# TheStageAI/TheWhisper

Measured on NVIDIA H100. Metric: tokens_per_sec, higher is better.
Workload: dtype bf16

## Files before the change

thewhisper_b200/csrc/api.cu:

```cuda
#include <limits.h>
#include <stdarg.h>
#include <stdlib.h>
#include <string.h>

#include <chrono>
#include <map>
#include <string>
#include <tuple>
#include <vector>

#ifdef BW_F16
#define BW_RENAME_SUFFIX _f16
#define BW_API_NS bw_api_f16
#else
#define BW_RENAME_SUFFIX _bf16
#define BW_API_NS bw_api
#endif
#include "abi_rename.h"
#include "../../include/thewhisper_b200.h"
#include "decode.cuh"
#include "decode_mega_common.cuh"
#include "kernels.h"

namespace BW_NS {

static thread_local char g_err[1024] = "";
void set_error(const char* fmt, ...) {
  va_list ap;
  va_start(ap, fmt);
  vsnprintf(g_err, sizeof(g_err), fmt, ap);
  va_end(ap);
}
const char* get_error() { return g_err; }
int g_pdl = 0;
static int g_pdl_enabled = -1;

size_t word_timestamps_work_floats(int Ha, int Tcap, int S);
int word_timestamps_batch_device(cudaStream_t st, const float* align, int Ha, int Tcap, int S, const int* items_dev, const int* slot_map_dev,
                                 int map_pitch, int n, int maxT, int maxNF, double time_precision, float* work, float* out_dev);

namespace {

struct EncLayer {
  const float *ln1g, *ln1b, *bqkv, *bo, *ln2g, *ln2b, *b1, *b2;
  const bf16 *wqkv, *wo, *w1, *w2;
};
constexpr const char* kDecQuant[6] = {"wqkv", "wo", "xwq", "xwo", "w1", "w2"};
struct DecLayer {
  const float *ln1g, *ln1b, *bqkv, *bo, *ln2g, *ln2b, *xbq, *xbv, *xbo, *ln3g, *ln3b, *b1, *b2;
  const void *wqkv, *wo, *xwq, *xwo, *w1, *w2;
  const bf16 *xwk, *xwv;
  const float* sc[6] = {nullptr, nullptr, nullptr, nullptr, nullptr, nullptr};
};

struct GraphKey {
  int A, G, begin_index, ts_rules, align, variant, eos, pad, ts_begin, no_ts, key_start, scores;
  bool operator<(const GraphKey& o) const {
    return std::tie(A, G, begin_index, ts_rules, align, variant, eos, pad, ts_begin, no_ts, key_start, scores) <
           std::tie(o.A, o.G, o.begin_index, o.ts_rules, o.align, o.variant, o.eos, o.pad, o.ts_begin, o.no_ts, o.key_start, o.scores);
  }
};

}
}

using namespace BW_NS;

struct bw_engine {
  bw_config cfg;
  std::map<std::string, const void*> tensors;
  bool finalized = false;
  int D, H, S, F, V, Vp, Tmax, Spad;
  const bf16 *conv1_w = nullptr, *conv2_w = nullptr;
  const void* embed = nullptr;
  const float* embed_scale = nullptr;
  const float** wscale_tab = nullptr;
  const float *conv1_b = nullptr, *conv2_b = nullptr, *enc_pos = nullptr, *enc_lnf_g = nullptr, *enc_lnf_b = nullptr;
  const float *dec_pos = nullptr, *dec_lnf_g = nullptr, *dec_lnf_b = nullptr;
  std::vector<EncLayer> enc;
  std::vector<DecLayer> dec;
  LogmelPlan* mel_plan = nullptr;
  std::vector<int> align_pairs;
  bf16 *mel_tm = nullptr, *h1 = nullptr, *xn = nullptr, *qkv = nullptr, *vt = nullptr, *ao = nullptr, *hbuf = nullptr, *enc_out = nullptr;
  float *x_enc = nullptr, *mel_scratch = nullptr;
  unsigned* mel_max = nullptr;
  bf16 *cross_k = nullptr, *cross_v = nullptr;
  bf16 *self_k = nullptr, *self_v = nullptr;
  int *tokens = nullptr, *finished = nullptr, *pos = nullptr, *anc = nullptr, *anc_tmp = nullptr, *head_slots = nullptr;
  unsigned *done_ctr = nullptr, *xcounters = nullptr, *sup_bits = nullptr, *bsup_bits = nullptr, *sel_ctr = nullptr;
  unsigned long long* sel_best = nullptr;
  float *dx = nullptr, *dqkv = nullptr, *dattn = nullptr, *dq = nullptr, *dh = nullptr, *logits = nullptr, *part_o = nullptr,
        *part_ml = nullptr, *align = nullptr, *lse = nullptr, *ts_work = nullptr, *ts_out = nullptr;
  int *reorder_tmp = nullptr, *cand_tokens = nullptr, *ts_items = nullptr, *ts_map = nullptr;
  float *run_scores = nullptr, *cand_scores = nullptr;
  size_t align_bytes = 0;
  int A = 0, G = 1, Q = 0;
  int steps = 0;
  bw_decode_opts opts{};
  bool use_anc = false;
  int* key_start = nullptr;
  bool has_k0 = false;
  bool scores = false;
  float *sc_lp = nullptr, *sc_lmass = nullptr, *sc_nsp = nullptr;
  int* nsp_cfg = nullptr;
  bool graph_pending = false;
  std::map<GraphKey, cudaGraphExec_t> graphs;
  std::map<GraphKey, long long> graph_used;
  long long graph_tick = 0, graph_captures = 0, graph_capture_us = 0, graph_evictions = 0;
  int max_graphs = 64;
  cudaGraphExec_t cur_graph = nullptr;
  std::map<cudaGraphExec_t, int> graph_kernels;
  long long step_kernel_launches = 0;
  bool no_graph = false, simt = false, no_mega = false, no_fused_select = false;
  int mega_flags = MEGA_DEFAULT_FLAGS;
  bf16 *dbn = nullptr, *dba = nullptr, *dbh = nullptr;
  float* dpart = nullptr;
  int batch_min = 3;
  bool gemm2 = true;
  bool attn_vdirect = true;
  long long gemm2_min_rows = 1024;
  bool enc_graph = true;
  bool enc_pdl = false;
  std::map<int, cudaGraphExec_t> enc_graphs;
  std::map<int, int> enc_calls;
  int num_sms = 132;
  int pf_rows = 0;
  long long pf_part_floats = 0;
  float *pf_x = nullptr, *pf_part = nullptr;
  bf16 *pf_n = nullptr, *pf_q = nullptr, *pf_a = nullptr, *pf_h = nullptr;
  unsigned* mega_bar = nullptr;
  long long* mega_trace = nullptr;
  std::map<std::string, std::pair<void*, size_t>> buffers;
};

namespace BW_API_NS {

template <typename T>
int dalloc(bw_engine* e, const char* name, T** p, size_t count, bool zero = true) {
  const size_t bytes = count * sizeof(T);
  BW_CUDA_OK(cudaMalloc(reinterpret_cast<void**>(p), bytes ? bytes : 16));
  if (zero) BW_CUDA_OK(cudaMemset(*p, 0, bytes ? bytes : 16));
  e->buffers[name] = std::make_pair(static_cast<void*>(*p), bytes);
  return 0;
}

template <typename T>
int need(bw_engine* e, const std::string& name, const T** out) {
  auto it = e->tensors.find(name);
  BW_CHECK(it != e->tensors.end() && it->second != nullptr, "weight '%s' is not bound", name.c_str());
  *out = static_cast<const T*>(it->second);
  return 0;
}

int gemm(bw_engine* e, cudaStream_t st, const GemmA& a, const bf16* W, int B, int rows, int N, int K, const GemmEpi& epi) {
  if (e->simt) return gemm_simt(st, a, W, B, rows, N, K, epi);
  if (e->gemm2 && a.kwrap >= K && a.pitch == K && a.batch_stride == (long long)rows * K && !epi.pos && gemm_tc2_supported(B * rows, N, K) &&
      (long long)B * rows >= e->gemm2_min_rows)
    return gemm_tc2(st, a.base, W, B * rows, N, K, rows, epi, 0);
  return gemm_tc(st, a, W, B, rows, N, K, epi, 0);
}

GemmA plainA(const bf16* base, int rows, int K) {
  GemmA a;
  a.base = base;
  a.batch_stride = (long long)rows * K;
  a.pitch = K;
  a.rows_base = rows;
  a.kwrap = INT_MAX;
  return a;
}

GemmEpi plainEpi(int rows, int ld) {
  GemmEpi ep;
  ep.batch_stride = (long long)rows * ld;
  ep.row_stride = ld;
  ep.head_stride = 64;
  return ep;
}

int encode_impl(bw_engine* e, int B, cudaStream_t st) {
  const int D = e->D, S = e->S, F = e->F, H = e->H, ffn = e->cfg.ffn, nm = e->cfg.n_mels;
  {
    GemmA a;
    a.base = e->mel_tm; a.batch_stride = (long long)(F + 2) * nm; a.pitch = nm; a.rows_base = F + 2; a.kwrap = nm;
    GemmEpi ep;
    ep.bias = e->conv1_b; ep.act = 1;
    ep.out_bf16 = e->h1 + D;
    ep.batch_stride = (long long)(F + 2) * D; ep.row_stride = D;
    if (int rc = gemm(e, st, a, e->conv1_w, B, F, D, 3 * nm, ep)) return rc;
  }
  {
    GemmA a;
    a.base = e->h1; a.batch_stride = (long long)(F + 2) * D; a.pitch = 2 * D; a.rows_base = (F + 2) / 2; a.kwrap = 2 * D;
    GemmEpi ep;
    ep.bias = e->conv2_b; ep.act = 1; ep.pos = e->enc_pos;
    ep.out_f32 = e->x_enc;
    ep.batch_stride = (long long)S * D; ep.row_stride = D;
    if (int rc = gemm(e, st, a, e->conv2_w, B, S, D, 3 * D, ep)) return rc;
  }
  const float scale = 0.125f;
  (void)scale;
  for (size_t l = 0; l < e->enc.size(); ++l) {
    const EncLayer& L = e->enc[l];
    if (int rc = layernorm_bf16(st, e->x_enc, L.ln1g, L.ln1b, e->xn, B * S, D)) return rc;
    {
      GemmEpi ep = plainEpi(S, 3 * D);
      ep.bias = L.bqkv; ep.out_bf16 = e->qkv;
      if (int rc = gemm(e, st, plainA(e->xn, S, D), L.wqkv, B, S, 3 * D, D, ep)) return rc;
    }
    if (e->simt) {
      if (int rc = attn_enc_simt(st, e->qkv, e->ao, B, S, H)) return rc;
    } else {
      if (e->attn_vdirect) {
        if (int rc = attn_enc_tc(st, e->qkv, nullptr, e->ao, B, S, e->Spad, H)) return rc;
      } else {
        if (int rc = transpose_v(st, e->qkv, e->vt, B, S, e->Spad, H)) return rc;
        if (int rc = attn_enc_tc(st, e->qkv, e->vt, e->ao, B, S, e->Spad, H)) return rc;
      }
    }
    {
      GemmEpi ep = plainEpi(S, D);
      ep.bias = L.bo; ep.residual = e->x_enc; ep.out_f32 = e->x_enc;
      if (int rc = gemm(e, st, plainA(e->ao, S, D), L.wo, B, S, D, D, ep)) return rc;
    }
    if (int rc = layernorm_bf16(st, e->x_enc, L.ln2g, L.ln2b, e->xn, B * S, D)) return rc;
    {
      GemmEpi ep = plainEpi(S, ffn);
      ep.bias = L.b1; ep.act = 1; ep.out_bf16 = e->hbuf;
      if (int rc = gemm(e, st, plainA(e->xn, S, D), L.w1, B, S, ffn, D, ep)) return rc;
    }
    {
      GemmEpi ep = plainEpi(S, D);
      ep.bias = L.b2; ep.residual = e->x_enc; ep.out_f32 = e->x_enc;
      if (int rc = gemm(e, st, plainA(e->hbuf, S, ffn), L.w2, B, S, D, ffn, ep)) return rc;
    }
  }
  if (int rc = layernorm_bf16(st, e->x_enc, e->enc_lnf_g, e->enc_lnf_b, e->enc_out, B * S, D)) return rc;
  const long long per_layer = (long long)e->cfg.max_audios * H * S * 64;
  for (size_t l = 0; l < e->dec.size(); ++l) {
    const DecLayer& L = e->dec[l];
    GemmEpi ep;
    ep.batch_stride = (long long)H * S * 64; ep.row_stride = 64; ep.head_stride = (long long)S * 64;
    ep.out_bf16 = e->cross_k + l * per_layer;
    if (int rc = gemm(e, st, plainA(e->enc_out, S, D), L.xwk, B, S, D, D, ep)) return rc;
    ep.bias = L.xbv;
    ep.out_bf16 = e->cross_v + l * per_layer;
    if (int rc = gemm(e, st, plainA(e->enc_out, S, D), L.xwv, B, S, D, D, ep)) return rc;
  }
  return 0;
}

constexpr int DPART_PER_ROW = 20480;

int step_batched_impl(bw_engine* e, cudaStream_t st);
int step_batched(bw_engine* e, cudaStream_t st) {
  if (g_pdl_enabled < 0) {
    const char* ev = getenv("BW_PDL");
    g_pdl_enabled = (ev && ev[0] == '0') ? 0 : 1;
  }
  g_pdl = g_pdl_enabled;
  const int rc = step_batched_impl(e, st);
  g_pdl = 0;
  return rc;
}
int step_batched_impl(bw_engine* e, cudaStream_t st) {
  const int D = e->D, H = e->H, S = e->S, ffn = e->cfg.ffn, Tmax = e->Tmax, Q = e->Q, A = e->A, G = e->G;
  const long long self_layer = (long long)e->cfg.max_audios * e->cfg.max_beams * Tmax * D;
  const long long cross_layer = (long long)e->cfg.max_audios * H * S * 64;
  const bool w8 = e->embed_scale != nullptr;
  auto proj = [&](const bf16* in, int K, const void* W, const float* sc, int N, int* ns) {
    const DecGemmPlan pl = gemm_dec_plan(Q, N, K, e->num_sms, true, w8);
    BW_CHECK((long long)pl.ksplit * N <= DPART_PER_ROW, "batched step: %d splits x N=%d exceed the partial-sum buffer", pl.ksplit, N);
    GemmEpi ep;
    ep.out_f32 = e->dpart; ep.row_stride = N;
    *ns = pl.ksplit;
    return gemm_dec(st, in, W, sc, Q, N, K, 0, ep, pl, (long long)Q * N);
  };
  if (int rc = launch_embed(st, e->embed, e->embed_scale, e->dec_pos, e->tokens, e->pos, e->dx, Q, D, Tmax)) return rc;
  int ns = 0;
  const float* pbias = nullptr;
  for (size_t l = 0; l < e->dec.size(); ++l) {
    const DecLayer& L = e->dec[l];
    bf16* kc = e->self_k + l * self_layer;
    bf16* vc = e->self_v + l * self_layer;
    if (int rc = launch_resid_ln(st, e->dx, e->dpart, ns, (long long)Q * D, pbias, L.ln1g, L.ln1b, e->dbn, Q, D)) return rc;
    if (int rc = proj(e->dbn, D, L.wqkv, L.sc[0], 3 * D, &ns)) return rc;
    {
      SelfAttnArgs s;
      s.qkv = e->dpart; s.nsplit = ns; s.split_stride = (long long)Q * 3 * D; s.qkv_bias = L.bqkv; s.q_alpha = 0.125f;
      s.kc = kc; s.vc = vc; s.kc_w = kc; s.vc_w = vc; s.anc = e->use_anc ? e->anc : nullptr; s.out_bf16 = e->dba; s.pos = e->pos;
      s.k0 = e->has_k0 ? e->key_start : nullptr;
      s.H = H; s.D = D; s.Tmax = Tmax;
      if (int rc = launch_self_attn(st, s, Q)) return rc;
    }
    if (int rc = proj(e->dba, D, L.wo, L.sc[1], D, &ns)) return rc;
    if (int rc = launch_resid_ln(st, e->dx, e->dpart, ns, (long long)Q * D, L.bo, L.ln2g, L.ln2b, e->dbn, Q, D)) return rc;
    if (int rc = proj(e->dbn, D, L.xwq, L.sc[2], D, &ns)) return rc;
    {
      CrossAttnArgs c;
      c.q = e->dpart; c.nsplit = ns; c.split_stride = (long long)Q * D; c.q_bias = L.xbq; c.q_alpha = 0.125f;
      c.kc = e->cross_k + l * cross_layer; c.vc = e->cross_v + l * cross_layer; c.out_bf16 = e->dba;
      c.part_o = e->part_o; c.part_ml = e->part_ml; c.counters = e->xcounters;
      c.S = S; c.H = H; c.D = D; c.G = G; c.pos = e->pos;
      if (e->opts.record_alignment && e->cfg.n_align_heads > 0) {
        c.align = e->align; c.head_slots = e->head_slots + l * H; c.Ha = e->cfg.n_align_heads;
        c.Tcap = e->cfg.max_align_steps; c.step_base = e->opts.begin_index;
      }
      if (int rc = launch_cross_attn(st, c, A)) return rc;
    }
    if (int rc = proj(e->dba, D, L.xwo, L.sc[3], D, &ns)) return rc;
    if (int rc = launch_resid_ln(st, e->dx, e->dpart, ns, (long long)Q * D, L.xbo, L.ln3g, L.ln3b, e->dbn, Q, D)) return rc;
    if (int rc = proj(e->dbn, D, L.w1, L.sc[4], ffn, &ns)) return rc;
    if (int rc = launch_gelu_bias(st, e->dpart, ns, (long long)Q * ffn, L.b1, e->dbh, Q, ffn)) return rc;
    if (int rc = proj(e->dbh, ffn, L.w2, L.sc[5], D, &ns)) return rc;
    pbias = L.b2;
  }
  if (int rc = launch_resid_ln(st, e->dx, e->dpart, ns, (long long)Q * D, pbias, e->dec_lnf_g, e->dec_lnf_b, e->dbn, Q, D)) return rc;
  {
    const DecGemmPlan pl = gemm_dec_plan(Q, e->V, D, e->num_sms, false, w8);
    GemmEpi ep;
    ep.out_f32 = e->logits; ep.row_stride = e->Vp;
    if (int rc = gemm_dec(st, e->dbn, e->embed, e->embed_scale, Q, e->V, D, e->V, ep, pl, 0)) return rc;
  }
  return 0;
}

constexpr int PREFILL_ROWS = 4096;

int prefill_pass(bw_engine* e, cudaStream_t st, int t0, int n) {
  const int D = e->D, H = e->H, S = e->S, ffn = e->cfg.ffn, Tmax = e->Tmax, Q = e->Q, R = e->Q * n;
  const long long self_layer = (long long)e->cfg.max_audios * e->cfg.max_beams * Tmax * D;
  const long long cross_layer = (long long)e->cfg.max_audios * H * S * 64;
  const bool w8 = e->embed_scale != nullptr;
  auto proj = [&](const bf16* in, int K, const void* W, const float* sc, int N, int* ns) {
    const DecGemmPlan pl = gemm_dec_plan(R, N, K, e->num_sms, true, w8);
    GemmEpi ep;
    ep.out_f32 = e->pf_part; ep.row_stride = N;
    *ns = pl.ksplit;
    return gemm_dec(st, in, W, sc, R, N, K, 0, ep, pl, (long long)R * N);
  };
  if (int rc = launch_prefill_embed(st, e->embed, e->embed_scale, e->dec_pos, e->tokens, e->pf_x, Q, n, t0, D, Tmax)) return rc;
  int ns = 0;
  const float* pbias = nullptr;
  for (size_t l = 0; l < e->dec.size(); ++l) {
    const DecLayer& L = e->dec[l];
    bf16* kc = e->self_k + l * self_layer;
    bf16* vc = e->self_v + l * self_layer;
    const bool last = l + 1 == e->dec.size();
    if (int rc = launch_resid_ln(st, e->pf_x, e->pf_part, ns, (long long)R * D, pbias, L.ln1g, L.ln1b, e->pf_n, R, D)) return rc;
    if (int rc = proj(e->pf_n, D, L.wqkv, L.sc[0], 3 * D, &ns)) return rc;
    if (int rc = launch_prefill_proj_sum(st, e->pf_part, ns, (long long)R * 3 * D, L.bqkv, 3 * D, D, R, last ? nullptr : e->pf_q, kc, vc, n,
                                         t0, Tmax))
      return rc;
    if (last) break;
    if (int rc = launch_prefill_self_attn(st, e->pf_q, kc, vc, e->pf_a, Q, n, t0, H, Tmax, e->has_k0 ? e->key_start : nullptr)) return rc;
    if (int rc = proj(e->pf_a, D, L.wo, L.sc[1], D, &ns)) return rc;
    if (int rc = launch_resid_ln(st, e->pf_x, e->pf_part, ns, (long long)R * D, L.bo, L.ln2g, L.ln2b, e->pf_n, R, D)) return rc;
    if (int rc = proj(e->pf_n, D, L.xwq, L.sc[2], D, &ns)) return rc;
    if (int rc = launch_prefill_proj_sum(st, e->pf_part, ns, (long long)R * D, L.xbq, D, D, R, e->pf_q, nullptr, nullptr, n, t0, Tmax)) return rc;
    if (int rc = launch_prefill_cross_attn(st, e->pf_q, e->cross_k + l * cross_layer, e->cross_v + l * cross_layer, e->pf_a, e->A, e->G, n, S, H))
      return rc;
    if (int rc = proj(e->pf_a, D, L.xwo, L.sc[3], D, &ns)) return rc;
    if (int rc = launch_resid_ln(st, e->pf_x, e->pf_part, ns, (long long)R * D, L.xbo, L.ln3g, L.ln3b, e->pf_n, R, D)) return rc;
    if (int rc = proj(e->pf_n, D, L.w1, L.sc[4], ffn, &ns)) return rc;
    if (int rc = launch_gelu_bias(st, e->pf_part, ns, (long long)R * ffn, L.b1, e->pf_h, R, ffn)) return rc;
    if (int rc = proj(e->pf_h, ffn, L.w2, L.sc[5], D, &ns)) return rc;
    pbias = L.b2;
  }
  return 0;
}

int prefill_fits(bw_engine* e, int R) {
  const int D = e->D, ffn = e->cfg.ffn;
  const int nk[4][2] = {{3 * D, D}, {D, D}, {ffn, D}, {D, ffn}};
  for (const auto& p : nk) {
    const DecGemmPlan pl = gemm_dec_plan(R, p[0], p[1], e->num_sms, true, e->embed_scale != nullptr);
    BW_CHECK((long long)pl.ksplit * R * p[0] <= e->pf_part_floats, "bw_decode_prefill: %d splits x %d rows x N=%d exceed the partial-sum buffer",
             pl.ksplit, R, p[0]);
  }
  return 0;
}

__global__ void set_pos_kernel(int* pos, int v) { *pos = v; }

int step_impl(bw_engine* e, cudaStream_t st) {
  const int D = e->D, H = e->H, S = e->S, ffn = e->cfg.ffn, V = e->V, Tmax = e->Tmax, Q = e->Q, A = e->A, G = e->G;
  const long long self_layer0 = (long long)e->cfg.max_audios * e->cfg.max_beams * Tmax * D;
  const long long cross_layer0 = (long long)e->cfg.max_audios * H * S * 64;
  bool mega_done = false, select_done = false;
  if (!e->no_mega && !e->has_k0 && G == 1 && Q <= 8 && (int)e->dec.size() <= MEGA_MAXL) {
    MegaArgs m{};
    for (size_t l = 0; l < e->dec.size(); ++l) {
      const DecLayer& L = e->dec[l];
      MegaLayer& o = m.layers[l];
      o.ln1g = L.ln1g; o.ln1b = L.ln1b; o.bqkv = L.bqkv; o.bo = L.bo; o.ln2g = L.ln2g; o.ln2b = L.ln2b; o.xbq = L.xbq; o.xbo = L.xbo;
      o.ln3g = L.ln3g; o.ln3b = L.ln3b; o.b1 = L.b1; o.b2 = L.b2;
      o.wqkv = L.wqkv; o.wo = L.wo; o.xwq = L.xwq; o.xwo = L.xwo; o.w1 = L.w1; o.w2 = L.w2;
      o.self_k = e->self_k + l * self_layer0; o.self_v = e->self_v + l * self_layer0;
      o.cross_k = e->cross_k + l * cross_layer0; o.cross_v = e->cross_v + l * cross_layer0;
      o.head_slots = (e->opts.record_alignment && e->cfg.n_align_heads > 0) ? e->head_slots + l * H : nullptr;
    }
    m.L = (int)e->dec.size(); m.D = D; m.H = H; m.ffn = ffn; m.V = V; m.S = S; m.Tmax = Tmax; m.Q = Q;
    m.embed = e->embed; m.embed_scale = e->embed_scale; m.wscale = e->wscale_tab; m.dec_pos = e->dec_pos; m.lnf_g = e->dec_lnf_g; m.lnf_b = e->dec_lnf_b;
    m.tokens = e->tokens; m.pos = e->pos; m.ldl = e->Vp;
    m.dx = e->dx; m.dqkv = e->dqkv; m.dattn = e->dattn; m.dq = e->dq; m.dh = e->dh; m.logits = e->logits;
    m.part_o = e->part_o; m.part_ml = e->part_ml; m.bar = e->mega_bar;
    int ns = e->num_sms / (Q * H);
    const int ns_min = (S + 255) / 256;
    if (ns < ns_min) ns = ns_min;
    if (ns > XSPLIT) ns = XSPLIT;
    m.nsplit = ns;
    if (e->opts.record_alignment && e->cfg.n_align_heads > 0) {
      m.align = e->align; m.Ha = e->cfg.n_align_heads; m.Tcap = e->cfg.max_align_steps; m.step_base = e->opts.begin_index;
    }
    m.trace = e->mega_trace;
    if (!e->opts.timestamp_rules && !e->no_fused_select && !e->scores) {
      m.fuse_select = 1;
      m.suppress_bits = e->sup_bits; m.begin_suppress_bits = e->bsup_bits; m.begin_index = e->opts.begin_index;
      m.eos = e->opts.eos_token; m.pad = e->opts.pad_token; m.finished = e->finished; m.tokens_rw = e->tokens; m.pos_rw = e->pos;
      m.sel_best = e->sel_best; m.sel_ctr = e->sel_ctr;
    }
    m.flags = e->mega_flags;
    const int rc = launch_decode_mega(st, m, e->num_sms);
    if (rc == 0) {
      mega_done = true;
      select_done = m.fuse_select != 0;
    }
    else if (rc != -3) return rc;
  }
  if (!mega_done && !e->simt && Q >= e->batch_min) {
    if (int rc = step_batched(e, st)) return rc;
    mega_done = true;
  }
  if (!mega_done) {
  if (int rc = launch_embed(st, e->embed, e->embed_scale, e->dec_pos, e->tokens, e->pos, e->dx, Q, D, Tmax)) return rc;
  const long long self_layer = (long long)e->cfg.max_audios * e->cfg.max_beams * Tmax * D;
  const long long cross_layer = (long long)e->cfg.max_audios * H * S * 64;
  for (size_t l = 0; l < e->dec.size(); ++l) {
    const DecLayer& L = e->dec[l];
    bf16* kc = e->self_k + l * self_layer;
    bf16* vc = e->self_v + l * self_layer;
    for (int m0 = 0; m0 < Q; m0 += Q) {
      GemvArgs g;
      g.M = Q - m0;
      g.x = e->dx + (long long)m0 * D; g.ldx = D; g.ln_g = L.ln1g; g.ln_b = L.ln1b;
      g.W = L.wqkv; g.wscale = L.sc[0]; g.N = 3 * D; g.K = D; g.bias = L.bqkv; g.alpha = 0.125f; g.alpha_cols = D;
      g.out = e->dqkv + (long long)m0 * 3 * D; g.ldo = 3 * D;
      g.kc = kc; g.vc = vc; g.D = D; g.Tmax = Tmax; g.seq0 = m0; g.pos = e->pos;
      if (int rc = launch_gemv(st, g)) return rc;
    }
    {
      SelfAttnArgs s;
      s.qkv = e->dqkv; s.kc = kc; s.vc = vc; s.anc = e->use_anc ? e->anc : nullptr; s.out = e->dattn; s.pos = e->pos;
      s.k0 = e->has_k0 ? e->key_start : nullptr;
      s.H = H; s.D = D; s.Tmax = Tmax;
      if (int rc = launch_self_attn(st, s, Q)) return rc;
    }
    for (int m0 = 0; m0 < Q; m0 += Q) {
      GemvArgs g;
      g.M = Q - m0;
      g.x = e->dattn + (long long)m0 * D; g.ldx = D; g.W = L.wo; g.wscale = L.sc[1]; g.N = D; g.K = D; g.bias = L.bo;
      g.residual = e->dx + (long long)m0 * D; g.out = e->dx + (long long)m0 * D; g.ldo = D;
      if (int rc = launch_gemv(st, g)) return rc;
    }
    for (int m0 = 0; m0 < Q; m0 += Q) {
      GemvArgs g;
      g.M = Q - m0;
      g.x = e->dx + (long long)m0 * D; g.ldx = D; g.ln_g = L.ln2g; g.ln_b = L.ln2b;
      g.W = L.xwq; g.wscale = L.sc[2]; g.N = D; g.K = D; g.bias = L.xbq; g.alpha = 0.125f; g.alpha_cols = D;
      g.out = e->dq + (long long)m0 * D; g.ldo = D;
      if (int rc = launch_gemv(st, g)) return rc;
    }
    {
      CrossAttnArgs c;
      c.q = e->dq; c.kc = e->cross_k + l * cross_layer; c.vc = e->cross_v + l * cross_layer; c.out = e->dattn;
      c.part_o = e->part_o; c.part_ml = e->part_ml; c.counters = e->xcounters;
      c.S = S; c.H = H; c.D = D; c.G = G; c.pos = e->pos;
      if (e->opts.record_alignment && e->cfg.n_align_heads > 0) {
        c.align = e->align; c.head_slots = e->head_slots + l * H; c.Ha = e->cfg.n_align_heads;
        c.Tcap = e->cfg.max_align_steps; c.step_base = e->opts.begin_index;
      }
      if (int rc = launch_cross_attn(st, c, A)) return rc;
    }
    for (int m0 = 0; m0 < Q; m0 += Q) {
      GemvArgs g;
      g.M = Q - m0;
      g.x = e->dattn + (long long)m0 * D; g.ldx = D; g.W = L.xwo; g.wscale = L.sc[3]; g.N = D; g.K = D; g.bias = L.xbo;
      g.residual = e->dx + (long long)m0 * D; g.out = e->dx + (long long)m0 * D; g.ldo = D;
      if (int rc = launch_gemv(st, g)) return rc;
    }
    for (int m0 = 0; m0 < Q; m0 += Q) {
      GemvArgs g;
      g.M = Q - m0;
      g.x = e->dx + (long long)m0 * D; g.ldx = D; g.ln_g = L.ln3g; g.ln_b = L.ln3b;
      g.W = L.w1; g.wscale = L.sc[4]; g.N = ffn; g.K = D; g.bias = L.b1; g.act = 1;
      g.out = e->dh + (long long)m0 * ffn; g.ldo = ffn;
      if (int rc = launch_gemv(st, g)) return rc;
    }
    for (int m0 = 0; m0 < Q; m0 += Q) {
      GemvArgs g;
      g.M = Q - m0;
      g.x = e->dh + (long long)m0 * ffn; g.ldx = ffn; g.W = L.w2; g.wscale = L.sc[5]; g.N = D; g.K = ffn; g.bias = L.b2;
      g.residual = e->dx + (long long)m0 * D; g.out = e->dx + (long long)m0 * D; g.ldo = D;
      if (int rc = launch_gemv(st, g)) return rc;
    }
  }
  for (int m0 = 0; m0 < Q; m0 += Q) {
    GemvArgs g;
    g.M = Q - m0;
    g.x = e->dx + (long long)m0 * D; g.ldx = D; g.ln_g = e->dec_lnf_g; g.ln_b = e->dec_lnf_b;
    g.W = e->embed; g.wscale = e->embed_scale; g.N = V; g.K = D;
    g.out = e->logits + (long long)m0 * e->Vp; g.ldo = e->Vp;
    if (int rc = launch_gemv(st, g)) return rc;
  }
  }
  if (select_done) return 0;
  SelectArgs s;
  s.logits = e->logits; s.V = V; s.ldl = e->Vp; s.Q = Q; s.Tmax = Tmax; s.tokens = e->tokens; s.finished = e->finished; s.pos = e->pos;
  s.done_ctr = e->done_ctr; s.suppress_bits = e->sup_bits; s.begin_suppress_bits = e->bsup_bits;
  s.begin_index = e->opts.begin_index; s.eos = e->opts.eos_token; s.pad = e->opts.pad_token;
  s.ts_rules = e->opts.timestamp_rules; s.ts_begin = e->opts.timestamp_begin; s.no_ts = e->opts.no_timestamps_token;
  s.max_initial_ts = e->opts.max_initial_timestamp_index; s.out_lse = e->lse;
  if (e->scores) { s.out_lp = e->sc_lp; s.out_lmass = e->sc_lmass; s.out_nsp = e->sc_nsp; s.nsp_cfg = e->nsp_cfg; }
  if (G > 1) { s.n_cand = 2 * G; s.run_scores = e->run_scores; s.cand_scores = e->cand_scores; s.cand_tokens = e->cand_tokens; }
  return launch_select(st, s);
}

__global__ void mel_to_tm_kernel(const float* __restrict__ mel, bf16* __restrict__ out, int n_mels, int frames) {
  __shared__ float tile[32][33];
  const int b = blockIdx.z, f0 = blockIdx.x * 32, m0 = blockIdx.y * 32;
  const int tx = threadIdx.x & 31, ty = threadIdx.x >> 5;
  for (int i = ty; i < 32; i += 8) {
    const int m = m0 + i, f = f0 + tx;
    tile[i][tx] = (m < n_mels && f < frames) ? mel[((long long)b * n_mels + m) * frames + f] : 0.f;
  }
  __syncthreads();
  for (int i = ty; i < 32; i += 8) {
    const int f = f0 + i, m = m0 + tx;
    if (f < frames && m < n_mels) out[((long long)b * (frames + 2) + f + 1) * n_mels + m] = f2e(tile[tx][i]);
  }
}

__global__ void iota_anc_kernel(int* anc, int Q, int Tmax) {
  const int i = blockIdx.x * blockDim.x + threadIdx.x;
  if (i < Q * Tmax) anc[i] = i / Tmax;
}

__global__ void reorder_kernel(const int* __restrict__ anc_old, int* __restrict__ anc_new, const int* __restrict__ tok_old,
                               int* __restrict__ tok_new, const int* __restrict__ parent, const int* __restrict__ next_tok,
                               const int* __restrict__ pos_ptr, int Tmax) {
  const int i = blockIdx.x;
  const int p = parent[i];
  const int cur = *pos_ptr;
  for (int s = threadIdx.x; s < Tmax; s += blockDim.x) {
    anc_new[i * Tmax + s] = (s < cur) ? anc_old[p * Tmax + s] : i;
    int t = tok_old[p * Tmax + s];
    if (s == cur) t = next_tok[i];
    tok_new[i * Tmax + s] = t;
  }
}

}
using namespace BW_API_NS;

extern "C" {

const char* bw_last_error(void) { return BW_NS::get_error(); }
int bw_abi_version(void) { return BW_ABI_VERSION; }
int bw_runtime_flags(void) { return (g_mega_coop == 1 ? 1 : 0) | (g_pdl_enabled == 1 ? 2 : 0); }
int bw_device_count(void) {
  int n = 0;
  if (cudaGetDeviceCount(&n) != cudaSuccess) {
    cudaGetLastError();
    return 0;
  }
  return n;
}

int bw_engine_create(const bw_config* cfg, bw_engine** out) {
  BW_CHECK(cfg && out, "bw_engine_create: null argument");
  BW_CHECK(cfg->d_model == cfg->n_heads * 64, "head_dim must be 64 (d_model=%d, heads=%d)", cfg->d_model, cfg->n_heads);
  BW_CHECK(cfg->d_model % 64 == 0 && cfg->ffn % 64 == 0, "d_model and ffn must be multiples of 64");
  BW_CHECK(cfg->n_mels == 128 || cfg->n_mels == 64, "n_mels=%d unsupported (the conv stem's TMA view needs a multiple of 64)", cfg->n_mels);
  BW_CHECK(cfg->max_beams >= 1 && cfg->max_beams <= MAXG, "max_beams must be in 1..%d", MAXG);
  BW_CHECK(cfg->max_source_positions >= 1 && cfg->max_source_positions <= 1536, "max_source_positions out of range (1..1536)");
  BW_CHECK(bw_device_count() > 0, "no CUDA device: thewhisper_b200 has no CPU fallback");
  bw_engine* e = new bw_engine();
  e->cfg = *cfg;
  e->D = cfg->d_model; e->H = cfg->n_heads; e->S = cfg->max_source_positions; e->F = 2 * e->S; e->V = cfg->vocab;
  e->Tmax = cfg->max_target_positions; e->Spad = (e->S + 7) / 8 * 8;
  e->Vp = (e->V + 31) / 32 * 32;
  {
    const char* bm = getenv("BW_BATCH_MIN");
    if (bm) e->batch_min = atoi(bm);
    const char* g2 = getenv("BW_GEMM2");
    if (g2) e->gemm2 = g2[0] != '0';
    const char* eg = getenv("BW_ENC_GRAPH");
    if (eg) e->enc_graph = eg[0] != '0';
    const char* ep = getenv("BW_ENC_PDL");
    if (ep) e->enc_pdl = ep[0] != '0';
    const char* avd = getenv("BW_ATTN_VDIRECT");
    if (avd) e->attn_vdirect = avd[0] != '0';
    const char* g2r = getenv("BW_GEMM2_MIN_ROWS");
    if (g2r) e->gemm2_min_rows = atoll(g2r);
  }
  const char* ng = getenv("BW_NO_GRAPH");
  e->no_graph = ng && ng[0] == '1';
  const char* nm = getenv("BW_NO_MEGA");
  e->no_mega = nm && nm[0] == '1';
  e->no_fused_select = getenv("BW_NO_FUSED_SELECT") != nullptr;
  {
    const char* sg = getenv("BW_STEP_GRAPHS");
    if (sg) e->max_graphs = atoi(sg);
  }
  {
    const char* fl = getenv("BW_MEGA_FLAGS");
    if (fl) e->mega_flags = atoi(fl);
  }
  {
    int dev = 0, sms = 132;
    if (cudaGetDevice(&dev) == cudaSuccess && cudaDeviceGetAttribute(&sms, cudaDevAttrMultiProcessorCount, dev) == cudaSuccess) e->num_sms = sms;
  }
  const char* impl = getenv("BW_GEMM_IMPL");
  e->simt = impl && strcmp(impl, "simt") == 0;
  *out = e;
  return 0;
}

void bw_engine_destroy(bw_engine* e) {
  if (!e) return;
  for (auto& kv : e->graphs) cudaGraphExecDestroy(kv.second);
  for (auto& kv : e->enc_graphs) cudaGraphExecDestroy(kv.second);
  for (auto& kv : e->buffers) cudaFree(kv.second.first);
  logmel_plan_destroy(e->mel_plan);
  delete e;
}

int bw_engine_set_tensor(bw_engine* e, const char* name, const void* p) {
  BW_CHECK(e && name && p, "bw_engine_set_tensor: null argument");
  BW_CHECK(!e->finalized, "bw_engine_set_tensor after finalize");
  e->tensors[name] = p;
  return 0;
}

int bw_engine_set_mel_filters(bw_engine* e, const float* bank_host) {
  BW_CHECK(e && bank_host, "bw_engine_set_mel_filters: null argument");
  logmel_plan_destroy(e->mel_plan);
  e->mel_plan = nullptr;
  return logmel_plan_create_from_bank(&e->mel_plan, bank_host, e->cfg.n_mels);
}

int bw_engine_set_alignment_heads(bw_engine* e, const int32_t* pairs, int32_t n) {
  BW_CHECK(e && (pairs || n == 0), "bw_engine_set_alignment_heads: null argument");
  BW_CHECK(n == e->cfg.n_align_heads, "alignment heads: got %d pairs, config says %d", n, e->cfg.n_align_heads);
  e->align_pairs.assign(pairs, pairs + 2 * n);
  return 0;
}

int bw_engine_finalize(bw_engine* e) {
  BW_CHECK(e && !e->finalized, "bw_engine_finalize: bad engine");
  const bw_config& c = e->cfg;
  const int D = e->D, S = e->S, F = e->F, H = e->H, V = e->V, Tmax = e->Tmax, A = c.max_audios, Qm = c.max_audios * c.max_beams;
#define NEED(T, field, name) if (int rc = need<T>(e, name, &field)) return rc;
  NEED(bf16, e->conv1_w, "enc.conv1.w") NEED(float, e->conv1_b, "enc.conv1.b")
  NEED(bf16, e->conv2_w, "enc.conv2.w") NEED(float, e->conv2_b, "enc.conv2.b")
  NEED(float, e->enc_pos, "enc.pos") NEED(float, e->enc_lnf_g, "enc.lnf.g") NEED(float, e->enc_lnf_b, "enc.lnf.b")
  NEED(void, e->embed, "dec.embed") NEED(float, e->dec_pos, "dec.pos")
  NEED(float, e->dec_lnf_g, "dec.lnf.g") NEED(float, e->dec_lnf_b, "dec.lnf.b")
  e->enc.resize(c.enc_layers);
  for (int i = 0; i < c.enc_layers; ++i) {
    const std::string p = "enc." + std::to_string(i) + ".";
    EncLayer& L = e->enc[i];
    NEED(float, L.ln1g, p + "ln1.g") NEED(float, L.ln1b, p + "ln1.b") NEED(bf16, L.wqkv, p + "wqkv") NEED(float, L.bqkv, p + "bqkv")
    NEED(bf16, L.wo, p + "wo") NEED(float, L.bo, p + "bo") NEED(float, L.ln2g, p + "ln2.g") NEED(float, L.ln2b, p + "ln2.b")
    NEED(bf16, L.w1, p + "w1") NEED(float, L.b1, p + "b1") NEED(bf16, L.w2, p + "w2") NEED(float, L.b2, p + "b2")
  }
  e->dec.resize(c.dec_layers);
  for (int i = 0; i < c.dec_layers; ++i) {
    const std::string p = "dec." + std::to_string(i) + ".";
    DecLayer& L = e->dec[i];
    NEED(float, L.ln1g, p + "ln1.g") NEED(float, L.ln1b, p + "ln1.b") NEED(void, L.wqkv, p + "wqkv") NEED(float, L.bqkv, p + "bqkv")
    NEED(void, L.wo, p + "wo") NEED(float, L.bo, p + "bo") NEED(float, L.ln2g, p + "ln2.g") NEED(float, L.ln2b, p + "ln2.b")
    NEED(void, L.xwq, p + "xwq") NEED(float, L.xbq, p + "xbq") NEED(bf16, L.xwk, p + "xwk") NEED(bf16, L.xwv, p + "xwv")
    NEED(float, L.xbv, p + "xbv") NEED(void, L.xwo, p + "xwo") NEED(float, L.xbo, p + "xbo")
    NEED(float, L.ln3g, p + "ln3.g") NEED(float, L.ln3b, p + "ln3.b")
    NEED(void, L.w1, p + "w1") NEED(float, L.b1, p + "b1") NEED(void, L.w2, p + "w2") NEED(float, L.b2, p + "b2")
  }
  {
    const bool w8 = e->tensors.count("dec.embed.scale") != 0;
    std::map<std::string, bool> want;
    if (w8) NEED(float, e->embed_scale, "dec.embed.scale")
    want["dec.embed.scale"] = true;
    for (int i = 0; i < c.dec_layers; ++i) {
      for (int k = 0; k < 6; ++k) {
        const std::string n = "dec." + std::to_string(i) + "." + kDecQuant[k] + ".scale";
        want[n] = true;
        if (w8) {
          BW_CHECK(e->tensors.count(n), "int8 decoder weights: scale '%s' is not bound ('dec.embed.scale' is)", n.c_str());
          NEED(float, e->dec[i].sc[k], n)
        }
      }
    }
    for (const auto& kv : e->tensors) {
      const std::string& n = kv.first;
      if (n.size() > 6 && n.compare(n.size() - 6, 6, ".scale") == 0) {
        BW_CHECK(want.count(n), "weight '%s': only the int8 decoder matrices (dec.embed, dec.<i>.{wqkv,wo,xwq,xwo,w1,w2}) have scales", n.c_str());
        BW_CHECK(w8, "scale '%s' is bound but 'dec.embed.scale' is not: int8 decoder weights need the scales of all seven kinds", n.c_str());
      }
    }
    if (w8) {
      std::vector<const float*> tab;
      for (const DecLayer& L : e->dec) tab.insert(tab.end(), L.sc, L.sc + 6);
      if (dalloc(e, "wscale_tab", &e->wscale_tab, tab.size())) return -1;
      BW_CUDA_OK(cudaMemcpy(e->wscale_tab, tab.data(), tab.size() * sizeof(const float*), cudaMemcpyHostToDevice));
    }
  }
#undef NEED
  BW_CHECK(e->mel_plan != nullptr, "mel filter bank not set (bw_engine_set_mel_filters)");
  const size_t BS = (size_t)A * S;
  if (dalloc(e, "mel_tm", &e->mel_tm, (size_t)A * (F + 2) * c.n_mels)) return -1;
  if (dalloc(e, "mel_scratch", &e->mel_scratch, (size_t)A * F * c.n_mels)) return -1;
  if (dalloc(e, "mel_max", &e->mel_max, (size_t)A)) return -1;
  if (dalloc(e, "h1", &e->h1, (size_t)A * (F + 2) * D)) return -1;
  if (dalloc(e, "x_enc", &e->x_enc, BS * D)) return -1;
  if (dalloc(e, "xn", &e->xn, BS * D)) return -1;
  if (dalloc(e, "qkv", &e->qkv, BS * 3 * D)) return -1;
  if (dalloc(e, "vt", &e->vt, (size_t)A * H * 64 * e->Spad)) return -1;
  if (dalloc(e, "ao", &e->ao, BS * D)) return -1;
  if (dalloc(e, "hbuf", &e->hbuf, BS * c.ffn)) return -1;
  if (dalloc(e, "enc_out", &e->enc_out, BS * D)) return -1;
  if (dalloc(e, "cross_k", &e->cross_k, (size_t)c.dec_layers * A * H * S * 64, false)) return -1;
  if (dalloc(e, "cross_v", &e->cross_v, (size_t)c.dec_layers * A * H * S * 64, false)) return -1;
  if (dalloc(e, "self_k", &e->self_k, (size_t)c.dec_layers * Qm * Tmax * D, false)) return -1;
  if (dalloc(e, "self_v", &e->self_v, (size_t)c.dec_layers * Qm * Tmax * D, false)) return -1;
  if (dalloc(e, "tokens", &e->tokens, (size_t)Qm * Tmax)) return -1;
  if (dalloc(e, "tokens_tmp", &e->reorder_tmp, (size_t)Qm * Tmax + 2 * Qm)) return -1;
  if (dalloc(e, "finished", &e->finished, (size_t)Qm)) return -1;
  if (dalloc(e, "pos", &e->pos, 1)) return -1;
  if (dalloc(e, "anc", &e->anc, (size_t)Qm * Tmax)) return -1;
  if (dalloc(e, "anc_tmp", &e->anc_tmp, (size_t)Qm * Tmax)) return -1;
  if (dalloc(e, "key_start", &e->key_start, (size_t)Qm)) return -1;
  if (dalloc(e, "done_ctr", &e->done_ctr, 1)) return -1;
  if (dalloc(e, "mega_bar", &e->mega_bar, 1024)) return -1;
  {
    const char* tr = getenv("BW_MEGA_TRACE");
    if (tr && tr[0] == '1' && dalloc(e, "mega_trace", &e->mega_trace, (size_t)e->num_sms * MEGA_TRACE_N * 6)) return -1;
  }
  if (dalloc(e, "xcounters", &e->xcounters, (size_t)A * H)) return -1;
  if (dalloc(e, "sel_ctr", &e->sel_ctr, 1)) return -1;
  if (dalloc(e, "sel_best", &e->sel_best, (size_t)Qm)) return -1;
  if (dalloc(e, "sup_bits", &e->sup_bits, (size_t)(V + 31) / 32)) return -1;
  if (dalloc(e, "bsup_bits", &e->bsup_bits, (size_t)(V + 31) / 32)) return -1;
  if (dalloc(e, "dx", &e->dx, (size_t)Qm * D)) return -1;
  if (dalloc(e, "dqkv", &e->dqkv, (size_t)Qm * 3 * D)) return -1;
  if (dalloc(e, "dattn", &e->dattn, (size_t)Qm * D)) return -1;
  if (dalloc(e, "dq", &e->dq, (size_t)Qm * D)) return -1;
  if (dalloc(e, "dh", &e->dh, (size_t)Qm * c.ffn)) return -1;
  if (dalloc(e, "logits", &e->logits, (size_t)Qm * e->Vp)) return -1;
  {
    const size_t qpad = ((size_t)Qm + 127) / 128 * 128;
    if (dalloc(e, "dbn", &e->dbn, qpad * D)) return -1;
    if (dalloc(e, "dba", &e->dba, qpad * D)) return -1;
    if (dalloc(e, "dbh", &e->dbh, qpad * c.ffn)) return -1;
    if (dalloc(e, "dpart", &e->dpart, (size_t)Qm * DPART_PER_ROW)) return -1;
  }
  if (dalloc(e, "lse", &e->lse, (size_t)Qm)) return -1;
  if (dalloc(e, "sc_lp", &e->sc_lp, (size_t)Qm * e->Tmax) || dalloc(e, "sc_lmass", &e->sc_lmass, (size_t)Qm * e->Tmax) ||
      dalloc(e, "sc_nsp", &e->sc_nsp, (size_t)Qm) || dalloc(e, "nsp_cfg", &e->nsp_cfg, 2))
    return -1;
  if (dalloc(e, "run_scores", &e->run_scores, (size_t)Qm)) return -1;
  if (dalloc(e, "cand_scores", &e->cand_scores, (size_t)Qm * 16)) return -1;
  if (dalloc(e, "cand_tokens", &e->cand_tokens, (size_t)Qm * 16)) return -1;
  if (dalloc(e, "part_o", &e->part_o, (size_t)A * H * XSPLIT * c.max_beams * 64)) return -1;
  if (dalloc(e, "part_ml", &e->part_ml, (size_t)A * H * XSPLIT * c.max_beams * 2)) return -1;
  if (dalloc(e, "head_slots", &e->head_slots, (size_t)c.dec_layers * H)) return -1;
  {
    std::vector<int> hs((size_t)c.dec_layers * H, -1);
    for (int i = 0; i < c.n_align_heads && 2 * i + 1 < (int)e->align_pairs.size(); ++i) {
      const int l = e->align_pairs[2 * i], h = e->align_pairs[2 * i + 1];
      BW_CHECK(l >= 0 && l < c.dec_layers && h >= 0 && h < H, "alignment head (%d,%d) out of range", l, h);
      hs[(size_t)l * H + h] = i;
    }
    BW_CUDA_OK(cudaMemcpy(e->head_slots, hs.data(), hs.size() * sizeof(int), cudaMemcpyHostToDevice));
  }
  if (c.n_align_heads > 0) {
    BW_CHECK((int)e->align_pairs.size() == 2 * c.n_align_heads, "alignment heads not set");
    if (dalloc(e, "align", &e->align, (size_t)Qm * c.n_align_heads * c.max_align_steps * S)) return -1;
    if (dalloc(e, "ts_map", &e->ts_map, (size_t)A * c.max_align_steps)) return -1;
    if (dalloc(e, "ts_work", &e->ts_work, (size_t)A * word_timestamps_work_floats(c.n_align_heads, c.max_align_steps, S), false)) return -1;
    if (dalloc(e, "ts_out", &e->ts_out, (size_t)A * (c.max_align_steps + 8))) return -1;
    if (dalloc(e, "ts_items", &e->ts_items, (size_t)A * 3)) return -1;
  }
  e->finalized = true;
  return 0;
}

int bw_engine_buffer(bw_engine* e, const char* name, void** p, size_t* bytes) {
  BW_CHECK(e && name && p, "bw_engine_buffer: null argument");
  auto it = e->buffers.find(name);
  BW_CHECK(it != e->buffers.end(), "bw_engine_buffer: unknown buffer '%s'", name);
  *p = it->second.first;
  if (bytes) *bytes = it->second.second;
  return 0;
}

int bw_logmel(bw_engine* e, const float* pcm, int32_t B, int32_t n_samples, float* mel_f32_out, void* stream) {
  BW_CHECK(e && e->finalized && pcm, "bw_logmel: bad arguments");
  BW_CHECK(B >= 1 && B <= e->cfg.max_audios, "bw_logmel: B=%d outside 1..%d", B, e->cfg.max_audios);
  BW_CHECK(n_samples == e->F * 160, "bw_logmel: n_samples=%d, expected %d for this chunk length", n_samples, e->F * 160);
  return logmel(static_cast<cudaStream_t>(stream), e->mel_plan, pcm, B, n_samples, e->F, e->mel_tm, mel_f32_out, e->mel_scratch, e->mel_max);
}

int bw_logmel_long(bw_engine* e, const float* pcm, int32_t B, int32_t n_samples, float* mel_f32_out, void* stream) {
  BW_CHECK(e && e->finalized && pcm && mel_f32_out, "bw_logmel_long: bad arguments");
  BW_CHECK(B >= 1 && B <= e->cfg.max_audios, "bw_logmel_long: B=%d outside 1..%d", B, e->cfg.max_audios);
  BW_CHECK(n_samples >= 400, "bw_logmel_long: n_samples=%d below one 400-sample frame", n_samples);
  return logmel_long(static_cast<cudaStream_t>(stream), e->mel_plan, pcm, B, n_samples, mel_f32_out, e->mel_max);
}

int bw_set_mel(bw_engine* e, const float* mel, int32_t B, void* stream) {
  BW_CHECK(e && e->finalized && mel, "bw_set_mel: bad arguments");
  BW_CHECK(B >= 1 && B <= e->cfg.max_audios, "bw_set_mel: B=%d outside 1..%d", B, e->cfg.max_audios);
  dim3 grid((e->F + 31) / 32, (e->cfg.n_mels + 31) / 32, B);
  mel_to_tm_kernel<<<grid, 256, 0, static_cast<cudaStream_t>(stream)>>>(mel, e->mel_tm, e->cfg.n_mels, e->F);
  BW_CUDA_OK(cudaGetLastError());
  return 0;
}

static int encode_pdl(bw_engine* e, int B, cudaStream_t st) {
  if (!e->enc_pdl) return encode_impl(e, B, st);
  if (g_pdl_enabled < 0) {
    const char* ev = getenv("BW_PDL");
    g_pdl_enabled = (ev && ev[0] == '0') ? 0 : 1;
  }
  g_pdl = g_pdl_enabled;
  const int rc = encode_impl(e, B, st);
  g_pdl = 0;
  return rc;
}

int bw_encode(bw_engine* e, int32_t B, void* stream) {
  BW_CHECK(e && e->finalized, "bw_encode: engine not finalized");
  BW_CHECK(B >= 1 && B <= e->cfg.max_audios, "bw_encode: B=%d outside 1..%d", B, e->cfg.max_audios);
  cudaStream_t st = static_cast<cudaStream_t>(stream);
  if (e->no_graph || !e->enc_graph || e->simt) return encode_pdl(e, B, st);
  auto it = e->enc_graphs.find(B);
  if (it == e->enc_graphs.end()) {
    if (e->enc_calls[B]++ == 0) return encode_pdl(e, B, st);
    cudaStream_t cs;
    BW_CUDA_OK(cudaStreamCreateWithFlags(&cs, cudaStreamNonBlocking));
    cudaGraph_t graph = nullptr;
    cudaGraphExec_t exec = nullptr;
    for (int attempt = 0; attempt < 2 && !exec; ++attempt) {
      BW_CUDA_OK(cudaStreamBeginCapture(cs, cudaStreamCaptureModeThreadLocal));
      const int rc = encode_pdl(e, B, cs);
      cudaError_t ce = cudaStreamEndCapture(cs, &graph);
      if (rc == 0 && ce == cudaSuccess) ce = cudaGraphInstantiate(&exec, graph, 0);
      if (graph) cudaGraphDestroy(graph);
      graph = nullptr;
      if (rc == 0 && ce == cudaSuccess) break;
      exec = nullptr;
      cudaGetLastError();
      if (attempt == 0 && g_pdl_enabled == 1) {
        g_pdl_enabled = 0;
        continue;
      }
      break;
    }
    cudaStreamDestroy(cs);
    if (!exec) {
      e->enc_graph = false;
      return encode_pdl(e, B, st);
    }
    it = e->enc_graphs.emplace(B, exec).first;
  }
  BW_CUDA_OK(cudaGraphLaunch(it->second, st));
  return 0;
}

int bw_decode_begin(bw_engine* e, int32_t A, int32_t G, const int32_t* prompt, int32_t plen, const bw_decode_opts* opts, void* stream) {
  return bw_decode_begin_key_start(e, A, G, prompt, plen, opts, nullptr, stream);
}

int bw_decode_begin_key_start(bw_engine* e, int32_t A, int32_t G, const int32_t* prompt, int32_t plen, const bw_decode_opts* opts,
                              const int32_t* key_start, void* stream) {
  BW_CHECK(e && e->finalized && prompt && opts, "bw_decode_begin: bad arguments");
  BW_CHECK(A >= 1 && A <= e->cfg.max_audios && G >= 1 && G <= e->cfg.max_beams, "bw_decode_begin: A=%d G=%d out of range", A, G);
  BW_CHECK(plen >= 1 && plen <= e->Tmax, "bw_decode_begin: prompt_len=%d out of range", plen);
  BW_CHECK(opts->begin_index >= 1 && opts->begin_index <= plen, "bw_decode_begin: begin_index=%d outside 1..prompt_len", opts->begin_index);
  bool has_k0 = false;
  if (key_start)
    for (int a = 0; a < A; ++a) {
      BW_CHECK(key_start[a] >= 0 && key_start[a] < opts->begin_index, "bw_decode_begin: key_start[%d]=%d outside 0..begin_index-1 = 0..%d", a,
               key_start[a], opts->begin_index - 1);
      has_k0 |= key_start[a] > 0;
    }
  cudaStream_t st = static_cast<cudaStream_t>(stream);
  e->A = A; e->G = G; e->Q = A * G; e->opts = *opts; e->use_anc = G > 1; e->steps = 0; e->has_k0 = has_k0;
  const int Q = e->Q, Tmax = e->Tmax, V = e->V;
  std::vector<int> k0v((size_t)Q, 0);
  if (has_k0) {
    for (int q = 0; q < Q; ++q) k0v[q] = key_start[q / G];
    BW_CUDA_OK(cudaMemcpyAsync(e->key_start, k0v.data(), sizeof(int) * Q, cudaMemcpyHostToDevice, st));
  }
  std::vector<int> tok((size_t)Q * Tmax, opts->pad_token);
  for (int q = 0; q < Q; ++q) memcpy(&tok[(size_t)q * Tmax], prompt + (size_t)q * plen, sizeof(int) * plen);
  BW_CUDA_OK(cudaMemcpyAsync(e->tokens, tok.data(), tok.size() * sizeof(int), cudaMemcpyHostToDevice, st));
  std::vector<unsigned> bits((V + 31) / 32, 0u), bbits((V + 31) / 32, 0u);
  for (int i = 0; i < opts->n_suppress; ++i) {
    const int t = opts->suppress_tokens[i];
    if (t >= 0 && t < V) bits[t >> 5] |= 1u << (t & 31);
  }
  for (int i = 0; i < opts->n_begin_suppress; ++i) {
    const int t = opts->begin_suppress_tokens[i];
    if (t >= 0 && t < V) bbits[t >> 5] |= 1u << (t & 31);
  }
  BW_CUDA_OK(cudaMemcpyAsync(e->sup_bits, bits.data(), bits.size() * sizeof(unsigned), cudaMemcpyHostToDevice, st));
  BW_CUDA_OK(cudaMemcpyAsync(e->bsup_bits, bbits.data(), bbits.size() * sizeof(unsigned), cudaMemcpyHostToDevice, st));
  BW_CUDA_OK(cudaMemsetAsync(e->finished, 0, sizeof(int) * Q, st));
  BW_CUDA_OK(cudaMemsetAsync(e->pos, 0, sizeof(int), st));
  BW_CUDA_OK(cudaMemsetAsync(e->done_ctr, 0, sizeof(unsigned), st));
  BW_CUDA_OK(cudaMemsetAsync(e->xcounters, 0, sizeof(unsigned) * e->cfg.max_audios * e->H, st));
  iota_anc_kernel<<<(Q * Tmax + 255) / 256, 256, 0, st>>>(e->anc, Q, Tmax);
  BW_CUDA_OK(cudaGetLastError());
  BW_CUDA_OK(cudaStreamSynchronize(st));
  e->cur_graph = nullptr;
  e->scores = false;
  e->graph_pending = !e->no_graph;
  return 0;
}

static int acquire_step_graph(bw_engine* e) {
  e->graph_pending = false;
  const bw_decode_opts* opts = &e->opts;
  const int A = e->A, G = e->G;
  {
    GraphKey key{A, G, opts->begin_index, opts->timestamp_rules * 4 + (opts->max_initial_timestamp_index + 1) * 8, opts->record_alignment,
                 e->mega_flags * 4 + (e->no_mega ? 1 : 0) + (e->no_fused_select ? 2 : 0),
                 opts->eos_token, opts->pad_token, opts->timestamp_begin, opts->no_timestamps_token, e->has_k0 ? 1 : 0, e->scores ? 1 : 0};
    auto it = e->graphs.find(key);
    if (it == e->graphs.end()) {
      while (e->max_graphs > 0 && (int)e->graphs.size() >= e->max_graphs) {
        auto lru = e->graph_used.begin();
        for (auto u = e->graph_used.begin(); u != e->graph_used.end(); ++u)
          if (u->second < lru->second) lru = u;
        auto g = e->graphs.find(lru->first);
        e->graph_kernels.erase(g->second);
        cudaGraphExecDestroy(g->second);
        e->graphs.erase(g);
        e->graph_used.erase(lru);
        ++e->graph_evictions;
      }
      const auto t_capture = std::chrono::steady_clock::now();
      cudaStream_t cs;
      BW_CUDA_OK(cudaStreamCreateWithFlags(&cs, cudaStreamNonBlocking));
      cudaGraph_t graph = nullptr;
      for (int attempt = 0; attempt < 2; ++attempt) {
        BW_CUDA_OK(cudaStreamBeginCapture(cs, cudaStreamCaptureModeThreadLocal));
        const int rc = step_impl(e, cs);
        const cudaError_t ce = cudaStreamEndCapture(cs, &graph);
        if (rc == 0 && ce == cudaSuccess) break;
        if (graph) cudaGraphDestroy(graph);
        graph = nullptr;
        cudaGetLastError();
        if (attempt == 0 && (g_mega_coop == 1 || g_pdl_enabled == 1)) {
          g_mega_coop = 0;
          g_pdl_enabled = 0;
          continue;
        }
        cudaStreamDestroy(cs);
        if (rc == 0) set_error("cudaStreamEndCapture: %s", cudaGetErrorString(ce));
        return -1;
      }
      int n_kernel_nodes = 0;
      {
        size_t nn = 0;
        if (cudaGraphGetNodes(graph, nullptr, &nn) == cudaSuccess && nn > 0) {
          std::vector<cudaGraphNode_t> nodes(nn);
          if (cudaGraphGetNodes(graph, nodes.data(), &nn) == cudaSuccess) {
            for (size_t i = 0; i < nn; ++i) {
              cudaGraphNodeType ty;
              if (cudaGraphNodeGetType(nodes[i], &ty) == cudaSuccess && ty == cudaGraphNodeTypeKernel) ++n_kernel_nodes;
            }
          }
        }
      }
      cudaGraphExec_t exec = nullptr;
      BW_CUDA_OK(cudaGraphInstantiate(&exec, graph, 0));
      cudaGraphDestroy(graph);
      e->graph_kernels[exec] = n_kernel_nodes;
      cudaStreamDestroy(cs);
      it = e->graphs.emplace(key, exec).first;
      ++e->graph_captures;
      e->graph_capture_us +=
          std::chrono::duration_cast<std::chrono::microseconds>(std::chrono::steady_clock::now() - t_capture).count();
    }
    e->graph_used[key] = ++e->graph_tick;
    e->cur_graph = it->second;
  }
  return 0;
}

int bw_decode_run(bw_engine* e, int32_t n_steps, void* stream) {
  BW_CHECK(e && e->finalized && e->Q > 0, "bw_decode_run: no decode in progress");
  BW_CHECK(n_steps >= 0 && n_steps <= e->Tmax - e->steps, "bw_decode_run: %d steps from position %d would run past the last position %d",
           n_steps, e->steps, e->Tmax - 1);
  cudaStream_t st = static_cast<cudaStream_t>(stream);
  if (n_steps > 0 && e->graph_pending)
    if (int rc = acquire_step_graph(e)) return rc;
  for (int i = 0; i < n_steps; ++i, ++e->steps) {
    if (e->cur_graph) {
      BW_CUDA_OK(cudaGraphLaunch(e->cur_graph, st));
      e->step_kernel_launches += e->graph_kernels[e->cur_graph];
    } else {
      if (int rc = step_impl(e, st)) return rc;
    }
  }
  return 0;
}

int bw_decode_prefill(bw_engine* e, int32_t n_positions, int32_t max_rows_per_pass, void* stream) {
  BW_CHECK(e && e->finalized && e->Q > 0, "bw_decode_prefill: no decode in progress");
  BW_CHECK(e->steps == 0, "bw_decode_prefill: %d decoder steps have run since bw_decode_begin; the prefill must come first", e->steps);
  BW_CHECK(n_positions >= 1 && n_positions <= e->opts.begin_index - 1, "bw_decode_prefill: n_positions=%d outside 1..begin_index-1 = 1..%d",
           n_positions, e->opts.begin_index - 1);
  BW_CHECK(max_rows_per_pass == 0 || max_rows_per_pass >= e->Q, "bw_decode_prefill: max_rows_per_pass=%d is below the %d sequences of one position",
           max_rows_per_pass, e->Q);
  const bw_config& c = e->cfg;
  if (!e->pf_h) {
    const long long qm = (long long)c.max_audios * c.max_beams;
    e->pf_rows = (int)(qm * e->Tmax < PREFILL_ROWS ? qm * e->Tmax : (qm > PREFILL_ROWS ? qm : PREFILL_ROWS));
    const size_t rows = (size_t)e->pf_rows;
    const int widest = c.ffn > 3 * e->D ? c.ffn : 3 * e->D;
    e->pf_part_floats = (long long)rows * widest > (long long)e->num_sms * 128 * 256 ? (long long)rows * widest : (long long)e->num_sms * 128 * 256;
    const char* names[5] = {"pf_x", "pf_part", "pf_n", "pf_q", "pf_a"};
    for (const char* nm : names) {
      auto it = e->buffers.find(nm);
      if (it != e->buffers.end()) {
        cudaFree(it->second.first);
        e->buffers.erase(it);
      }
    }
    if (dalloc(e, "pf_x", &e->pf_x, rows * e->D, false) || dalloc(e, "pf_part", &e->pf_part, (size_t)e->pf_part_floats, false) ||
        dalloc(e, "pf_n", &e->pf_n, rows * e->D, false) || dalloc(e, "pf_q", &e->pf_q, rows * e->D, false) ||
        dalloc(e, "pf_a", &e->pf_a, rows * e->D, false) || dalloc(e, "pf_h", &e->pf_h, rows * c.ffn, false))
      return -1;
  }
  cudaStream_t st = static_cast<cudaStream_t>(stream);
  const int rows = (max_rows_per_pass > 0 && max_rows_per_pass < e->pf_rows) ? max_rows_per_pass : e->pf_rows;
  const int per = rows / e->Q;
  for (int t0 = 0; t0 < n_positions; t0 += per)
    if (int rc = prefill_fits(e, e->Q * (n_positions - t0 < per ? n_positions - t0 : per))) return rc;
  for (int t0 = 0; t0 < n_positions; t0 += per) {
    const int n = n_positions - t0 < per ? n_positions - t0 : per;
    if (int rc = prefill_pass(e, st, t0, n)) return rc;
  }
  set_pos_kernel<<<1, 1, 0, st>>>(e->pos, n_positions);
  BW_CUDA_OK(cudaGetLastError());
  e->steps = n_positions;
  return 0;
}

int bw_decode_scores_enable(bw_engine* e, int32_t nospeech_pos, int32_t nospeech_token, void* stream) {
  BW_CHECK(e && e->finalized && e->Q > 0, "bw_decode_scores_enable: no decode in progress");
  BW_CHECK(e->steps == 0, "bw_decode_scores_enable: a step or prefill has run since bw_decode_begin; scores must be enabled before it");
  BW_CHECK(nospeech_pos >= -1 && nospeech_pos <= e->opts.begin_index - 1, "bw_decode_scores_enable: nospeech_pos=%d outside -1..begin_index-1 = -1..%d",
           nospeech_pos, e->opts.begin_index - 1);
  BW_CHECK(nospeech_token >= 0 && nospeech_token < e->V, "bw_decode_scores_enable: nospeech_token=%d outside 0..%d", nospeech_token, e->V - 1);
  cudaStream_t st = static_cast<cudaStream_t>(stream);
  const int cfg[2] = {nospeech_pos, nospeech_token};
  BW_CUDA_OK(cudaMemcpyAsync(e->nsp_cfg, cfg, sizeof(cfg), cudaMemcpyHostToDevice, st));
  BW_CUDA_OK(cudaMemsetAsync(e->sc_lp, 0, sizeof(float) * e->Q * e->Tmax, st));
  BW_CUDA_OK(cudaMemsetAsync(e->sc_lmass, 0, sizeof(float) * e->Q * e->Tmax, st));
  BW_CUDA_OK(cudaMemsetAsync(e->sc_nsp, 0, sizeof(float) * e->Q, st));
  BW_CUDA_OK(cudaStreamSynchronize(st));
  e->scores = true;
  return 0;
}

int bw_decode_read_scores(bw_engine* e, float* lp_host, float* lmass_host, float* nsp_host, void* stream) {
  BW_CHECK(e && e->finalized && e->Q > 0 && e->scores, "bw_decode_read_scores: no decode with scores in progress");
  cudaStream_t st = static_cast<cudaStream_t>(stream);
  const size_t n = (size_t)e->Q * e->Tmax;
  if (lp_host) BW_CUDA_OK(cudaMemcpyAsync(lp_host, e->sc_lp, sizeof(float) * n, cudaMemcpyDeviceToHost, st));
  if (lmass_host) BW_CUDA_OK(cudaMemcpyAsync(lmass_host, e->sc_lmass, sizeof(float) * n, cudaMemcpyDeviceToHost, st));
  if (nsp_host) BW_CUDA_OK(cudaMemcpyAsync(nsp_host, e->sc_nsp, sizeof(float) * e->Q, cudaMemcpyDeviceToHost, st));
  BW_CUDA_OK(cudaStreamSynchronize(st));
  return 0;
}

long long bw_decode_kernel_launches(bw_engine* e) { return e ? e->step_kernel_launches : -1; }

int bw_decode_graph_stats(bw_engine* e, int64_t* out) {
  BW_CHECK(e && out, "bw_decode_graph_stats: bad arguments");
  out[0] = e->graph_captures;
  out[1] = e->graph_capture_us;
  out[2] = (int64_t)e->graphs.size();
  out[3] = e->graph_evictions;
  return 0;
}

int bw_decode_read(bw_engine* e, int32_t* tokens_host, int32_t* finished_host, int32_t* pos_host, void* stream) {
  BW_CHECK(e && e->finalized && e->Q > 0, "bw_decode_read: no decode in progress");
  cudaStream_t st = static_cast<cudaStream_t>(stream);
  if (tokens_host) BW_CUDA_OK(cudaMemcpyAsync(tokens_host, e->tokens, sizeof(int) * e->Q * e->Tmax, cudaMemcpyDeviceToHost, st));
  if (finished_host) BW_CUDA_OK(cudaMemcpyAsync(finished_host, e->finished, sizeof(int) * e->Q, cudaMemcpyDeviceToHost, st));
  if (pos_host) BW_CUDA_OK(cudaMemcpyAsync(pos_host, e->pos, sizeof(int), cudaMemcpyDeviceToHost, st));
  BW_CUDA_OK(cudaStreamSynchronize(st));
  return 0;
}

int bw_decode_reorder(bw_engine* e, const int32_t* parent_host, const int32_t* next_token_host, void* stream) {
  BW_CHECK(e && e->finalized && e->Q > 0 && parent_host && next_token_host, "bw_decode_reorder: bad arguments");
  cudaStream_t st = static_cast<cudaStream_t>(stream);
  const int Q = e->Q, Tmax = e->Tmax;
  int* d_parent = e->reorder_tmp + (size_t)e->cfg.max_audios * e->cfg.max_beams * Tmax;
  int* d_next = d_parent + Q;
  BW_CUDA_OK(cudaMemcpyAsync(d_parent, parent_host, sizeof(int) * Q, cudaMemcpyHostToDevice, st));
  BW_CUDA_OK(cudaMemcpyAsync(d_next, next_token_host, sizeof(int) * Q, cudaMemcpyHostToDevice, st));
  reorder_kernel<<<Q, 128, 0, st>>>(e->anc, e->anc_tmp, e->tokens, e->reorder_tmp, d_parent, d_next, e->pos, Tmax);
  BW_CUDA_OK(cudaGetLastError());
  BW_CUDA_OK(cudaMemcpyAsync(e->anc, e->anc_tmp, sizeof(int) * Q * Tmax, cudaMemcpyDeviceToDevice, st));
  BW_CUDA_OK(cudaMemcpyAsync(e->tokens, e->reorder_tmp, sizeof(int) * Q * Tmax, cudaMemcpyDeviceToDevice, st));
  BW_CUDA_OK(cudaStreamSynchronize(st));
  return 0;
}

int bw_decode_beam_step(bw_engine* e, const float* run_scores_host, float* cand_scores_host, int32_t* cand_tokens_host, void* stream) {
  BW_CHECK(e && e->finalized && e->Q > 0 && e->G > 1, "bw_decode_beam_step: no beam decode in progress");
  BW_CHECK(run_scores_host && cand_scores_host && cand_tokens_host, "bw_decode_beam_step: null pointer");
  cudaStream_t st = static_cast<cudaStream_t>(stream);
  const int Q = e->Q, nc = 2 * e->G;
  BW_CUDA_OK(cudaMemcpyAsync(e->run_scores, run_scores_host, sizeof(float) * Q, cudaMemcpyHostToDevice, st));
  if (int rc = bw_decode_run(e, 1, stream)) return rc;
  BW_CUDA_OK(cudaMemcpyAsync(cand_scores_host, e->cand_scores, sizeof(float) * Q * nc, cudaMemcpyDeviceToHost, st));
  BW_CUDA_OK(cudaMemcpyAsync(cand_tokens_host, e->cand_tokens, sizeof(int) * Q * nc, cudaMemcpyDeviceToHost, st));
  BW_CUDA_OK(cudaStreamSynchronize(st));
  return 0;
}

static int word_timestamps_impl(bw_engine* e, int32_t n, const int32_t* audio, const int32_t* slot_map, int32_t map_pitch, const int32_t* n_tokens,
                                const int32_t* num_frames, double time_precision, float* out_host, int32_t out_pitch, void* stream) {
  BW_CHECK(e && e->finalized && (audio || slot_map) && n_tokens && num_frames && out_host, "bw_word_timestamps: bad arguments");
  BW_CHECK(e->cfg.n_align_heads > 0 && e->align, "bw_word_timestamps: engine built without alignment heads");
  BW_CHECK(n >= 1 && n <= e->cfg.max_audios, "bw_word_timestamps: n=%d outside 1..%d", n, e->cfg.max_audios);
  const int Tcap = e->cfg.max_align_steps, Qm = e->cfg.max_audios * e->cfg.max_beams;
  std::vector<int> items((size_t)n * 3), map;
  int maxT = 0, maxNF = 0;
  for (int i = 0; i < n; ++i) {
    BW_CHECK(n_tokens[i] >= 1 && n_tokens[i] <= Tcap, "bw_word_timestamps: n_tokens=%d outside 1..%d", n_tokens[i], Tcap);
    BW_CHECK(num_frames[i] >= 1 && num_frames[i] <= e->S, "bw_word_timestamps: num_frames=%d outside 1..%d", num_frames[i], e->S);
    BW_CHECK(out_pitch >= n_tokens[i] + 1, "bw_word_timestamps: out_pitch=%d too small for %d tokens", out_pitch, n_tokens[i]);
    if (audio) BW_CHECK(audio[i] >= 0 && audio[i] < Qm, "bw_word_timestamps: slot index out of range");
    items[3 * i] = audio ? audio[i] : 0; items[3 * i + 1] = n_tokens[i]; items[3 * i + 2] = num_frames[i];
    maxT = n_tokens[i] > maxT ? n_tokens[i] : maxT;
    maxNF = num_frames[i] > maxNF ? num_frames[i] : maxNF;
  }
  cudaStream_t st = static_cast<cudaStream_t>(stream);
  if (slot_map) {
    BW_CHECK(map_pitch >= maxT, "bw_word_timestamps_gather: map_pitch=%d smaller than %d tokens", map_pitch, maxT);
    map.assign((size_t)n * Tcap, 0);
    for (int i = 0; i < n; ++i)
      for (int t = 0; t < n_tokens[i]; ++t) {
        const int sl = slot_map[(size_t)i * map_pitch + t];
        BW_CHECK(sl >= 0 && sl < Qm, "bw_word_timestamps_gather: slot %d out of range", sl);
        map[(size_t)i * Tcap + t] = sl;
      }
    BW_CUDA_OK(cudaMemcpyAsync(e->ts_map, map.data(), map.size() * sizeof(int), cudaMemcpyHostToDevice, st));
  }
  BW_CUDA_OK(cudaMemcpyAsync(e->ts_items, items.data(), items.size() * sizeof(int), cudaMemcpyHostToDevice, st));
  if (int rc = word_timestamps_batch_device(st, e->align, e->cfg.n_align_heads, Tcap, e->S, e->ts_items, slot_map ? e->ts_map : nullptr, Tcap, n, maxT,
                                            maxNF, time_precision, e->ts_work, e->ts_out))
    return rc;
  BW_CUDA_OK(cudaMemcpy2DAsync(out_host, (size_t)out_pitch * sizeof(float), e->ts_out, (size_t)(Tcap + 8) * sizeof(float),
                               (size_t)(maxT + 1) * sizeof(float), n, cudaMemcpyDeviceToHost, st));
  BW_CUDA_OK(cudaStreamSynchronize(st));
  return 0;
}

int bw_word_timestamps_batch(bw_engine* e, int32_t n, const int32_t* audio, const int32_t* n_tokens, const int32_t* num_frames,
                             double time_precision, float* out_host, int32_t out_pitch, void* stream) {
  BW_CHECK(audio, "bw_word_timestamps_batch: null argument");
  return word_timestamps_impl(e, n, audio, nullptr, 0, n_tokens, num_frames, time_precision, out_host, out_pitch, stream);
}

int bw_word_timestamps_gather(bw_engine* e, int32_t n, const int32_t* slot_map, int32_t map_pitch, const int32_t* n_tokens,
                              const int32_t* num_frames, double time_precision, float* out_host, int32_t out_pitch, void* stream) {
  BW_CHECK(slot_map, "bw_word_timestamps_gather: null argument");
  return word_timestamps_impl(e, n, nullptr, slot_map, map_pitch, n_tokens, num_frames, time_precision, out_host, out_pitch, stream);
}

int bw_word_timestamps(bw_engine* e, int32_t audio, int32_t n_tokens, int32_t num_frames, double time_precision, float* out_host,
                       void* stream) {
  return bw_word_timestamps_batch(e, 1, &audio, &n_tokens, &num_frames, time_precision, out_host, n_tokens + 1, stream);
}

int bw_op_gemm(const void* A, const void* W, int32_t M, int32_t N, int32_t K, const float* bias, float alpha, int32_t act,
               const float* residual, void* out, int32_t out_is_f32, int32_t impl, int32_t force_bn, void* stream) {
  BW_CHECK(A && W && out, "bw_op_gemm: null pointer");
  GemmEpi ep = plainEpi(M, N);
  ep.bias = bias; ep.alpha = alpha; ep.act = act; ep.residual = residual;
  if (out_is_f32) ep.out_f32 = static_cast<float*>(out);
  else ep.out_bf16 = static_cast<bf16*>(out);
  const GemmA a = plainA(static_cast<const bf16*>(A), M, K);
  cudaStream_t st = static_cast<cudaStream_t>(stream);
  if (impl == 1) return gemm_simt(st, a, static_cast<const bf16*>(W), 1, M, N, K, ep);
  if (impl == 2) return gemm_tc2(st, static_cast<const bf16*>(A), static_cast<const bf16*>(W), M, N, K, M, ep, force_bn);
  return gemm_tc(st, a, static_cast<const bf16*>(W), 1, M, N, K, ep, force_bn);
}

int bw_op_gemm_splitk(const void* A, const void* W, int32_t M, int32_t N, int32_t K, int32_t n_valid, int32_t ksplit, int32_t force_bn,
                      float* out_partials, int32_t* ksplit_used, void* stream) {
  BW_CHECK(A && W && out_partials && ksplit_used, "bw_op_gemm_splitk: null pointer");
  GemmEpi ep = plainEpi(M, N);
  ep.out_f32 = out_partials;
  ep.n_valid = (n_valid > 0 && n_valid < N) ? n_valid : 0;
  *ksplit_used = gemm_tc_ksplit(K, ksplit);
  return gemm_tc_split(static_cast<cudaStream_t>(stream), plainA(static_cast<const bf16*>(A), M, K), static_cast<const bf16*>(W), 1, M, N, K, ep,
                       force_bn, ksplit, (long long)M * N);
}

int bw_op_gemm_dec(const void* X, const void* W, int32_t Q, int32_t N, int32_t K, int32_t n_valid, int32_t want_split, float* out_partials,
                   int32_t* ksplit_used, void* stream) {
  BW_CHECK(X && W && out_partials && ksplit_used, "bw_op_gemm_dec: null pointer");
  int dev = 0, sms = 132;
  if (cudaGetDevice(&dev) == cudaSuccess) cudaDeviceGetAttribute(&sms, cudaDevAttrMultiProcessorCount, dev);
  const DecGemmPlan pl = gemm_dec_plan(Q, N, K, sms, want_split != 0);
  *ksplit_used = pl.ksplit;
  GemmEpi ep;
  ep.out_f32 = out_partials; ep.row_stride = N;
  return gemm_dec(static_cast<cudaStream_t>(stream), static_cast<const bf16*>(X), W, nullptr, Q, N, K, n_valid, ep, pl, (long long)Q * N);
}

int bw_op_gelu_bias(const float* partials, int32_t nsplit, const float* bias, void* h_bf16, int32_t Q, int32_t N, void* stream) {
  BW_CHECK(partials && bias && h_bf16 && nsplit >= 1, "bw_op_gelu_bias: bad arguments");
  return launch_gelu_bias(static_cast<cudaStream_t>(stream), partials, nsplit, (long long)Q * N, bias, static_cast<bf16*>(h_bf16), Q, N);
}

int bw_op_resid_ln(float* x, const float* partials, int32_t nsplit, const float* bias, const float* ln_g, const float* ln_b, void* y_bf16,
                   int32_t Q, int32_t D, void* stream) {
  BW_CHECK(x && (nsplit == 0 || partials) && (!y_bf16 || (ln_g && ln_b)), "bw_op_resid_ln: null pointer");
  return launch_resid_ln(static_cast<cudaStream_t>(stream), x, partials, nsplit, (long long)Q * D, bias, ln_g, ln_b, static_cast<bf16*>(y_bf16), Q, D);
}

int bw_op_attn_enc(const void* qkv, void* vt_scratch, void* out, int32_t B, int32_t S, int32_t H, int32_t impl, void* stream) {
  BW_CHECK(qkv && out, "bw_op_attn_enc: null pointer");
  cudaStream_t st = static_cast<cudaStream_t>(stream);
  if (impl == 1) return attn_enc_simt(st, static_cast<const bf16*>(qkv), static_cast<bf16*>(out), B, S, H);
  BW_CHECK(vt_scratch, "bw_op_attn_enc: vt_scratch required for the tensor-core path");
  const int Spad = (S + 7) / 8 * 8;
  if (impl == 3) return attn_enc_tc(st, static_cast<const bf16*>(qkv), nullptr, static_cast<bf16*>(out), B, S, Spad, H);
  if (int rc = transpose_v(st, static_cast<const bf16*>(qkv), static_cast<bf16*>(vt_scratch), B, S, Spad, H)) return rc;
  return attn_enc_tc(st, static_cast<const bf16*>(qkv), static_cast<const bf16*>(vt_scratch), static_cast<bf16*>(out), B, S, Spad, H);
}

int bw_op_layernorm(const float* x, const float* g, const float* b, void* out, int32_t out_is_f32, int32_t rows, int32_t D, void* stream) {
  BW_CHECK(x && g && b && out, "bw_op_layernorm: null pointer");
  cudaStream_t st = static_cast<cudaStream_t>(stream);
  return out_is_f32 ? layernorm_f32(st, x, g, b, static_cast<float*>(out), rows, D)
                    : layernorm_bf16(st, x, g, b, static_cast<bf16*>(out), rows, D);
}

int bw_op_gemv(const float* x, const float* ln_g, const float* ln_b, const void* W, int32_t M, int32_t N, int32_t K, const float* bias,
               float alpha, int32_t act, const float* residual, float* out, void* stream) {
  BW_CHECK(x && W && out, "bw_op_gemv: null pointer");
  GemvArgs g;
  g.x = x; g.ldx = K; g.ln_g = ln_g; g.ln_b = ln_b; g.W = static_cast<const bf16*>(W); g.N = N; g.K = K; g.M = M;
  g.bias = bias; g.alpha = alpha; g.alpha_cols = (alpha != 1.0f) ? N : 0; g.act = act; g.residual = residual; g.out = out; g.ldo = N;
  return launch_gemv(static_cast<cudaStream_t>(stream), g);
}

static int mega_plan(int32_t Q, int32_t D, int32_t ffn, int32_t num_sms, int32_t smem_optin, int32_t static_smem, int64_t* out, int esz) {
  BW_CHECK(out && Q >= 1 && D > 0 && ffn > 0 && num_sms > 0 && smem_optin > static_smem, "bw_op_mega_plan: bad arguments");
  int p0_off = 0;
  const size_t smem = mega::mega_smem_plan(Q <= 1 ? 1 : 2, D, ffn, num_sms, true, (size_t)(smem_optin - static_smem), &p0_off, esz);
  out[0] = (int64_t)smem;
  out[1] = p0_off;
  return smem ? 0 : -3;
}

int bw_op_mega_plan(int32_t Q, int32_t D, int32_t ffn, int32_t num_sms, int32_t smem_optin, int32_t static_smem, int64_t* out) {
  return mega_plan(Q, D, ffn, num_sms, smem_optin, static_smem, out, 2);
}

int bw_op_mega_plan_w8(int32_t Q, int32_t D, int32_t ffn, int32_t num_sms, int32_t smem_optin, int32_t static_smem, int64_t* out) {
  return mega_plan(Q, D, ffn, num_sms, smem_optin, static_smem, out, 1);
}

}
```

thewhisper_b200/csrc/decode.cuh:

```cuda
#pragma once
#include "common.cuh"

namespace BW_NS {

struct GemvArgs {
  const float* x = nullptr;
  int ldx = 0;
  const float* ln_g = nullptr;
  const float* ln_b = nullptr;
  const void* W = nullptr;
  const float* wscale = nullptr;
  int N = 0, K = 0, M = 0;
  const float* bias = nullptr;
  float alpha = 1.0f;
  int alpha_cols = 0;
  int act = 0;
  const float* residual = nullptr;
  float* out = nullptr;
  int ldo = 0;
  bf16* kc = nullptr;
  bf16* vc = nullptr;
  int D = 0, Tmax = 0, seq0 = 0;
  const int* pos = nullptr;
};

struct SelfAttnArgs {
  const float* qkv = nullptr;
  const bf16* kc = nullptr;
  const bf16* vc = nullptr;
  const int* anc = nullptr;
  float* out = nullptr;
  bf16* out_bf16 = nullptr;
  const int* pos = nullptr;
  const int* k0 = nullptr;
  int H = 0, D = 0, Tmax = 0;
  bf16* kc_w = nullptr;
  bf16* vc_w = nullptr;
  int nsplit = 0;
  long long split_stride = 0;
  const float* qkv_bias = nullptr;
  float q_alpha = 1.0f;
};

constexpr int XSPLIT = 12;
constexpr int MAXG = 8;

struct CrossAttnArgs {
  const float* q = nullptr;
  const bf16* kc = nullptr;
  const bf16* vc = nullptr;
  float* out = nullptr;
  bf16* out_bf16 = nullptr;
  float* part_o = nullptr;
  float* part_ml = nullptr;
  unsigned* counters = nullptr;
  int S = 0, H = 0, D = 0, G = 1;
  float* align = nullptr;
  int align_slot = -1;
  const int* head_slots = nullptr;
  int Ha = 0, Tcap = 0, step_base = 0;
  const int* pos = nullptr;
  int nsplit = 0;
  long long split_stride = 0;
  const float* q_bias = nullptr;
  float q_alpha = 1.0f;
};

struct SelectArgs {
  const float* logits = nullptr;
  int V = 0, Q = 0, Tmax = 0, ldl = 0;
  int* tokens = nullptr;
  int* finished = nullptr;
  int* pos = nullptr;
  unsigned* done_ctr = nullptr;
  const unsigned* suppress_bits = nullptr;
  const unsigned* begin_suppress_bits = nullptr;
  int begin_index = 0;
  int eos = 0, pad = 0;
  int ts_rules = 0, ts_begin = 0, no_ts = 0, max_initial_ts = -1;
  float* out_lse = nullptr;
  float* out_lp = nullptr;
  float* out_lmass = nullptr;
  float* out_nsp = nullptr;
  const int* nsp_cfg = nullptr;
  int n_cand = 0;
  const float* run_scores = nullptr;
  float* cand_scores = nullptr;
  int* cand_tokens = nullptr;
};

struct MegaLayer {
  const float *ln1g, *ln1b, *bqkv, *bo, *ln2g, *ln2b, *xbq, *xbo, *ln3g, *ln3b, *b1, *b2;
  const void *wqkv, *wo, *xwq, *xwo, *w1, *w2;
  bf16 *self_k, *self_v;
  const bf16 *cross_k, *cross_v;
  const int* head_slots;
};

constexpr int MEGA_MAXL = 32;
constexpr int MEGA_DEFAULT_FLAGS = 64;
constexpr int MEGA_TRACE_N = 264;

struct MegaArgs {
  MegaLayer layers[MEGA_MAXL];
  int L, D, H, ffn, V, S, Tmax, Q;
  int ldl;
  const void* embed;
  const float* dec_pos;
  const float *lnf_g, *lnf_b;
  const int* tokens;
  const int* pos;
  float *dx, *dqkv, *dattn, *dq, *dh, *logits;
  float *part_o, *part_ml;
  unsigned* bar;
  int nsplit;
  float* align;
  int Ha, Tcap, step_base;
  long long* trace;
  int flags;
  int fuse_select;
  const unsigned* suppress_bits;
  const unsigned* begin_suppress_bits;
  int begin_index, eos, pad;
  int* finished;
  int* tokens_rw;
  int* pos_rw;
  unsigned long long* sel_best;
  unsigned* sel_ctr;
  int p0_off;
  const float* const* wscale;
  const float* embed_scale;
};

int launch_decode_mega(cudaStream_t st, const MegaArgs& a, int num_sms);
extern int g_mega_coop;
int launch_gemv(cudaStream_t st, const GemvArgs& a);
int launch_embed(cudaStream_t st, const void* E, const float* Es, const float* P, const int* tokens, const int* pos, float* x, int Q, int D, int Tmax);
int launch_self_attn(cudaStream_t st, const SelfAttnArgs& a, int Q);
int launch_cross_attn(cudaStream_t st, const CrossAttnArgs& a, int A);
int launch_select(cudaStream_t st, const SelectArgs& a);
int launch_resid_ln(cudaStream_t st, float* x, const float* part, int nsplit, long long split_stride, const float* bias, const float* g,
                    const float* b, bf16* y, int Q, int D);


int launch_prefill_embed(cudaStream_t st, const void* E, const float* Es, const float* P, const int* tokens, float* x, int Q, int n, int t0,
                         int D, int Tmax);
int launch_prefill_proj_sum(cudaStream_t st, const float* part, int nsplit, long long split_stride, const float* bias, int N, int D, int R,
                            bf16* qout, bf16* kc, bf16* vc, int n, int t0, int Tmax);
int launch_prefill_self_attn(cudaStream_t st, const bf16* q, const bf16* kc, const bf16* vc, bf16* out, int Q, int n, int t0, int H, int Tmax,
                             const int* k0 = nullptr);
int launch_prefill_cross_attn(cudaStream_t st, const bf16* q, const bf16* kc, const bf16* vc, bf16* out, int A, int G, int n, int S, int H);

}
```

thewhisper_b200/csrc/decode_mega.cu:

```cuda
#include "decode_mega_common.cuh"

namespace BW_NS {

namespace {

using namespace mega;


constexpr unsigned V_NOTRACE = 1;

__device__ __noinline__ void wait_timeout(const char* what, unsigned a0, unsigned a1) {
  printf("[bw] decode_mega: %s timed out (block %d thread %d: %u %u)\n", what, blockIdx.x, threadIdx.x, a0, a1);
  __trap();
}
template <unsigned VAR>
struct GridBar {
  static constexpr bool TRACE = !(VAR & V_NOTRACE);
  unsigned* ctr;
  unsigned nblocks;
  unsigned epoch;
  long long* trace;
  __device__ __forceinline__ void arrive() {
    if (threadIdx.x == MT - 1) {
      if (TRACE && trace && epoch < MEGA_TRACE_N) trace[((long long)blockIdx.x * MEGA_TRACE_N + epoch) * 2] = global_ns();
      red_release_add(ctr, 1u);
    }
  }
  __device__ __forceinline__ void wait() {
    if (threadIdx.x == MT - 1) {
      const unsigned target = (epoch + 1) * nblocks;
      if (ld_acquire_u32(ctr) < target) {
        const long long t0 = clock64();
        while (ld_acquire_u32(ctr) < target) {
          if (clock64() - t0 > (1ll << 32)) {
            printf("[bw] decode_mega: grid barrier %u timed out (block %d)\n", epoch, blockIdx.x);
            __trap();
          }
        }
      }
      if (TRACE && trace && epoch < MEGA_TRACE_N) trace[((long long)blockIdx.x * MEGA_TRACE_N + epoch) * 2 + 1] = global_ns();
    }
    ++epoch;
    __syncthreads();
  }
  __device__ __forceinline__ void sync() {
    __syncthreads();
    arrive();
    wait();
  }
};

struct GemvDesc {
  const uint8_t* W;
  const float* scale;
  const float* bias;
  int N, K, R;
  int n0, nend;
  bool lm;
  const float* src;
  const float *lng, *lnb;
  float* out;
  int ldo;
  const float* residual;
  int act;
  float alpha;
  int alpha_cols;
  bf16 *kc, *vc;
};

__device__ __forceinline__ void split_rows(GemvDesc& d) {
  const int rc = (d.N + (int)gridDim.x - 1) / (int)gridDim.x;
  d.R = (rc + MW - 1) / MW;
  d.n0 = min(d.N, (int)blockIdx.x * rc);
  d.nend = min(d.N, d.n0 + rc);
}
template <unsigned VAR, bool W8>
__device__ __forceinline__ GemvDesc make_desc(const MegaArgs& a, const MegaLayer* layers, int l, int g, int pos) {
  GemvDesc d;
  d.scale = nullptr;
  if constexpr (W8) d.scale = l >= a.L ? a.embed_scale : a.wscale[l * 6 + g];
  d.lng = d.lnb = nullptr;
  d.residual = nullptr;
  d.act = 0;
  d.alpha = 1.f;
  d.alpha_cols = 0;
  d.kc = d.vc = nullptr;
  d.N = d.K = d.ldo = a.D;
  d.lm = false;
  if (l >= a.L) {
    d.W = static_cast<const uint8_t*>(a.embed); d.bias = nullptr; d.N = a.V; d.R = 2; d.n0 = 0; d.nend = a.V; d.lm = true; d.src = a.dx; d.lng = a.lnf_g; d.lnb = a.lnf_b; d.out = a.logits; d.ldo = a.ldl;
    return d;
  }
  const MegaLayer& L = layers[l];
  switch (g) {
    case 0:
      d.W = static_cast<const uint8_t*>(L.wqkv); d.bias = L.bqkv; d.N = 3 * a.D; d.src = a.dx; d.lng = L.ln1g; d.lnb = L.ln1b; d.out = a.dqkv; d.ldo = 3 * a.D;
      d.alpha = 0.125f; d.alpha_cols = a.D; d.kc = L.self_k; d.vc = L.self_v;
      break;
    case 1:
      d.W = static_cast<const uint8_t*>(L.wo); d.bias = L.bo; d.src = a.dattn; d.out = a.dx; d.residual = a.dx;
      break;
    case 2:
      d.W = static_cast<const uint8_t*>(L.xwq); d.bias = L.xbq; d.src = a.dx; d.lng = L.ln2g; d.lnb = L.ln2b; d.out = a.dq; d.alpha = 0.125f; d.alpha_cols = a.D;
      break;
    case 3:
      d.W = static_cast<const uint8_t*>(L.xwo); d.bias = L.xbo; d.src = a.part_o; d.out = a.dx; d.residual = a.dx;
      break;
    case 4:
      d.W = static_cast<const uint8_t*>(L.w1); d.bias = L.b1; d.N = a.ffn; d.src = a.dx; d.lng = L.ln3g; d.lnb = L.ln3b; d.out = a.dh; d.ldo = a.ffn; d.act = 1;
      break;
    default:
      d.W = static_cast<const uint8_t*>(L.w2); d.bias = L.b2; d.K = a.ffn; d.src = a.dh; d.out = a.dx; d.residual = a.dx;
      break;
  }
  split_rows(d);
  return d;
}

struct Pre {
  float bias;
  float scale;
  float4 g, b;
};

template <int ESZ>
__device__ __forceinline__ void issue_slabs(const GemvDesc& d, uint8_t* region, uint64_t* cbar) {
  if (threadIdx.x == DMA_T && d.n0 < d.nend) {
    const uint32_t bytes = (uint32_t)(d.nend - d.n0) * d.K * ESZ;
    mbar_arrive_expect_tx(cbar, bytes);
    if constexpr (ESZ == 2) bulk_g2s(region, reinterpret_cast<const bf16*>(d.W) + (long long)d.n0 * d.K, bytes, cbar);
    else bulk_g2s(region, d.W + (long long)d.n0 * d.K, bytes, cbar);
  }
}

template <bool W8>
__device__ __forceinline__ void prefetch_phase(const GemvDesc& d, Pre& p, uint8_t* pool, uint64_t* wbar, int gw, int warp, int lane) {
  constexpr int ESZ = W8 ? 1 : 2;
  int n;
  if (d.lm) {
    n = gw * d.R;
    if (n < d.N) issue_rows<ESZ>(pool + (size_t)warp * d.R * d.K * ESZ, wbar, d.W, d.K, d.R, n, d.N, lane);
  } else {
    n = d.n0 + warp * d.R;
  }
  const int r_sel = lane >> 3;
  p.bias = (d.bias && (lane & 7) < 2 && r_sel < d.R && n + r_sel < d.nend) ? d.bias[n + r_sel] : 0.f;
  if constexpr (W8) p.scale = (!d.lm && (lane & 7) < 2 && r_sel < d.R && n + r_sel < d.nend) ? d.scale[n + r_sel] : 1.f;
  const int k = threadIdx.x * 4;
  if (d.lng && k < d.K) {
    p.g = *reinterpret_cast<const float4*>(d.lng + k);
    p.b = *reinterpret_cast<const float4*>(d.lnb + k);
  }
}

template <int MB>
__device__ __forceinline__ void merge_xattn(float* xs, const GemvDesc& d, const MegaArgs& a, int M) {
  constexpr int XC = 6;
  static_assert(MAXD <= (MT - 32) * 4 && XSPLIT <= 16, "one float4 per staging thread and sequence; one lane per split");
  const int K = d.K, nsplit = a.nsplit;
  const int k = threadIdx.x * 4, sp_l = threadIdx.x & 15;
  const bool have = k < K;
#pragma unroll 1
  for (int m = 0; m < MB; ++m) {
    const int hb = (m * a.H + (k >> 6)) * nsplit;
    const float* po_base = a.part_o + hb * 64 + (k & 63);
    const bool live = have && m < M;
    float pm = -INFINITY, pl = 0.f;
    float4 po[XC];
    if (live && sp_l < nsplit) {
      const float2 v = __ldcg(reinterpret_cast<const float2*>(a.part_ml) + hb + sp_l);
      pm = v.x;
      pl = v.y;
    }
#pragma unroll
    for (int sp = 0; sp < XC; ++sp) {
      po[sp] = make_float4(0.f, 0.f, 0.f, 0.f);
      if (live && sp < nsplit) po[sp] = __ldcg(reinterpret_cast<const float4*>(po_base + sp * 64));
    }
    if (m == 0) asm volatile("bar.arrive 2, %0;" ::"n"(MT) : "memory");
    float mx = pl > 0.f ? pm : -INFINITY;
#pragma unroll
    for (int s = 8; s >= 1; s >>= 1) mx = fmaxf(mx, __shfl_xor_sync(0xffffffffu, mx, s));
    float lsum = 0.f;
    float4 o = make_float4(0.f, 0.f, 0.f, 0.f);
    for (int sp0 = 0;;) {
#pragma unroll
      for (int sp = 0; sp < XC; ++sp) {
        const float sm = __shfl_sync(0xffffffffu, pm, sp0 + sp, 16), sl = __shfl_sync(0xffffffffu, pl, sp0 + sp, 16);
        if (sp0 + sp < nsplit && sl > 0.f) {
          const float w = __expf(sm - mx);
          lsum = fmaf(sl, w, lsum);
          o.x = fmaf(po[sp].x, w, o.x);
          o.y = fmaf(po[sp].y, w, o.y);
          o.z = fmaf(po[sp].z, w, o.z);
          o.w = fmaf(po[sp].w, w, o.w);
        }
      }
      sp0 += XC;
      if (sp0 >= nsplit) break;
#pragma unroll
      for (int sp = 0; sp < XC; ++sp)
        if (live && sp0 + sp < nsplit) po[sp] = __ldcg(reinterpret_cast<const float4*>(po_base + (sp0 + sp) * 64));
    }
    if (!have) continue;
    float4 v = make_float4(0.f, 0.f, 0.f, 0.f);
    if (m < M) {
      v = make_float4(o.x / lsum, o.y / lsum, o.z / lsum, o.w / lsum);
      float* row = a.dattn + m * K;
      if (k >= d.n0 && k < d.nend) row[k] = v.x;
      if (k + 1 >= d.n0 && k + 1 < d.nend) row[k + 1] = v.y;
      if (k + 2 >= d.n0 && k + 2 < d.nend) row[k + 2] = v.z;
      if (k + 3 >= d.n0 && k + 3 < d.nend) row[k + 3] = v.w;
    }
    *reinterpret_cast<float4*>(xs + m * K + k) = v;
  }
}

__device__ __forceinline__ void stage_sync() { asm volatile("bar.sync 1, %0;" ::"n"(MT - 32) : "memory"); }
__device__ __forceinline__ void stage_done_stagers() {
  asm volatile("bar.sync 1, %0;" ::"n"(MT - 32) : "memory");
  asm volatile("bar.arrive 3, %0;" ::"n"(MT) : "memory");
}
__device__ __forceinline__ void stage_done_dma() { asm volatile("bar.sync 3, %0;" ::"n"(MT) : "memory"); }

template <int MB, unsigned VAR, class Dma>
__device__ __forceinline__ void stage_x(float* xs, float* red, const GemvDesc& d, const Pre& p, int M, bool split_end, const MegaArgs& a,
                                        bool xattn, Dma&& dma) {
  const int K = d.K;
  const int warp = threadIdx.x >> 5, lane = threadIdx.x & 31;
  if (warp == MW - 1) {
    if (xattn) asm volatile("bar.sync 2, %0;" ::"n"(MT) : "memory");
    dma();
    if (split_end) stage_done_dma();
    else __syncthreads();
    return;
  }
  if (xattn) {
    merge_xattn<MB>(xs, d, a, M);
    if (split_end) stage_done_stagers();
    else __syncthreads();
    return;
  }
  constexpr int ST = MT - 32;
  if (!d.lng) {
    constexpr int U = 4;
    for (int base = threadIdx.x * 4; base < MB * K; base += ST * 4 * U) {
      float4 v[U];
#pragma unroll
      for (int u = 0; u < U; ++u) {
        const int i = base + u * ST * 4;
        const int m = (MB > 1 && i >= K) ? 1 : 0;
        v[u] = make_float4(0.f, 0.f, 0.f, 0.f);
        if (i < MB * K && m < M) v[u] = __ldcg(reinterpret_cast<const float4*>(d.src + (long long)m * K + (i - m * K)));
      }
#pragma unroll
      for (int u = 0; u < U; ++u) {
        const int i = base + u * ST * 4;
        if (i < MB * K) *reinterpret_cast<float4*>(xs + i) = v[u];
      }
    }
    if (split_end) stage_done_stagers();
    else __syncthreads();
    return;
  }
  const int k = threadIdx.x * 4;
  const bool have = k < K;
  float4 v[MB];
#pragma unroll
  for (int m = 0; m < MB; ++m) {
    v[m] = make_float4(0.f, 0.f, 0.f, 0.f);
    if (have && m < M) v[m] = __ldcg(reinterpret_cast<const float4*>(d.src + (long long)m * K + k));
  }
#pragma unroll
  for (int m = 0; m < MB; ++m) {
    const float s = warp_sum((v[m].x + v[m].y) + (v[m].z + v[m].w));
    if (lane == 0) red[m * MW + warp] = s;
  }
  stage_sync();
  float mean[MB];
#pragma unroll
  for (int m = 0; m < MB; ++m) {
    float s = 0.f;
#pragma unroll
    for (int w = 0; w < MW - 1; ++w) s += red[m * MW + w];
    mean[m] = s / (float)K;
    float ss = 0.f;
    if (have) {
      const float a0 = v[m].x - mean[m], a1 = v[m].y - mean[m], a2 = v[m].z - mean[m], a3 = v[m].w - mean[m];
      ss = (a0 * a0 + a1 * a1) + (a2 * a2 + a3 * a3);
    }
    ss = warp_sum(ss);
    if (lane == 0) red[(MB + m) * MW + warp] = ss;
  }
  stage_sync();
#pragma unroll
  for (int m = 0; m < MB; ++m) {
    float ss = 0.f;
#pragma unroll
    for (int w = 0; w < MW - 1; ++w) ss += red[(MB + m) * MW + w];
    const float rstd = rsqrtf(ss / (float)K + 1e-5f);
    if (have) {
      float4 o;
      o.x = (v[m].x - mean[m]) * rstd * p.g.x + p.b.x;
      o.y = (v[m].y - mean[m]) * rstd * p.g.y + p.b.y;
      o.z = (v[m].z - mean[m]) * rstd * p.g.z + p.b.z;
      o.w = (v[m].w - mean[m]) * rstd * p.g.w + p.b.w;
      *reinterpret_cast<float4*>(xs + m * K + k) = o;
    }
  }
  if (split_end) stage_done_stagers();
  else __syncthreads();
}

template <int MB, unsigned VAR, bool W8>
__device__ __forceinline__ void finish_rows(const GemvDesc& d, const float (&acc)[RMAX][MB], float scale, float bias, int n, int M,
                                            float res, bool res_valid, int D, int Tmax, int pos, int lane) {
  const int m = lane & 7, r_sel = lane >> 3;
  const int nn = n + r_sel;
  if (r_sel < d.R && m < MB && m < M && nn < d.nend) {
    float v = 0.f;
#pragma unroll
    for (int r = 0; r < RMAX; ++r) {
#pragma unroll
      for (int mm = 0; mm < MB; ++mm)
        if (r == r_sel && mm == m) v = acc[r][mm];
    }
    if (W8) v *= scale;
    v += bias;
    if (nn < d.alpha_cols) v *= d.alpha;
    if (d.act == 1) v = gelu_erf(v);
    if (d.residual) v += res_valid ? res : __ldcg(d.residual + (long long)m * d.ldo + nn);
    d.out[(long long)m * d.ldo + nn] = v;
    if (d.kc && nn >= D) {
      const long long row = ((long long)m * Tmax + pos) * D;
      if (nn < 2 * D) d.kc[row + nn - D] = f2e(v);
      else d.vc[row + nn - 2 * D] = f2e(v);
    }
  }
}

template <int MB, unsigned VAR, bool W8>
__global__ void __launch_bounds__(MT, 1) decode_mega_kernel(const __grid_constant__ MegaArgs a) {
  constexpr bool TRACE = !(VAR & V_NOTRACE);
  constexpr int ESZ = W8 ? 1 : 2;
  extern __shared__ __align__(128) uint8_t dyn[];
  float* red = reinterpret_cast<float*>(dyn);
  float* xs = red + 64;
  uint8_t* pool = reinterpret_cast<uint8_t*>(xs + (size_t)MB * a.ffn);
  uint8_t* att = pool + ATT_OFF;
  __shared__ __align__(8) uint64_t wbar[2 * MW];
  __shared__ __align__(8) uint64_t xbar;
  __shared__ __align__(8) uint64_t cbar[2];
  __shared__ long long wts[MW][2];
  __shared__ __align__(16) MegaLayer sl[MEGA_MAXL];

  const int warp = threadIdx.x >> 5, lane = threadIdx.x & 31;
  const int gw = blockIdx.x * MW + warp, GW = gridDim.x * MW;
  const int D = a.D, H = a.H, Q = a.Q;
  const int pos0 = *a.pos;
  GridBar<VAR> bar{a.bar, gridDim.x, 0u, a.trace};
  const bool split_end = (a.flags & 64) != 0;
  long long* const mkbase = (TRACE && a.trace) ? a.trace + (long long)gridDim.x * MEGA_TRACE_N * 2 + (long long)blockIdx.x * MEGA_TRACE_N * 4 : nullptr;
  auto mark = [&](int j) {
    if (mkbase && threadIdx.x == 0 && bar.epoch < MEGA_TRACE_N) mkbase[bar.epoch * 4 + j] = global_ns();
  };

  const int nsplit = a.nsplit;
  const int ks = (a.S + nsplit - 1) / nsplit;
  const int grp = threadIdx.x >> 3, sub = threadIdx.x & 7;
  uint32_t wpar = 0, wpar1 = 0, xpar = 0, cpar0 = 0, cpar1 = 0;

  {
    static_assert(sizeof(MegaLayer) % 8 == 0, "MegaLayer is copied in 8-byte words");
    const unsigned long long* src = reinterpret_cast<const unsigned long long*>(a.layers);
    unsigned long long* dst = reinterpret_cast<unsigned long long*>(sl);
    for (int i = threadIdx.x; i < a.L * (int)(sizeof(MegaLayer) / 8); i += MT) dst[i] = src[i];
  }
  if (threadIdx.x == 0) {
    for (int i = 0; i < 2 * MW; ++i) mbar_init(&wbar[i], 1);
    mbar_init(&xbar, 1);
    mbar_init(&cbar[0], 1);
    mbar_init(&cbar[1], 1);
    fence_mbar_init();
  }
  __syncthreads();

  const int pos = pos0;
  GemvDesc cur = make_desc<VAR, W8>(a, sl, 0, 0, pos);
  Pre pre;
  const bool dbuf = a.p0_off > 0;
  issue_slabs<ESZ>(cur, pool + a.p0_off, &cbar[0]);
  prefetch_phase<W8>(cur, pre, pool, &wbar[warp], gw, warp, lane);
  if (blockIdx.x == 0) {
    for (int i = threadIdx.x; i < Q * D; i += MT) {
      const int q = i / D, d = i - q * D;
      const int tok = a.tokens[q * a.Tmax + pos];
      if constexpr (W8)
        a.dx[i] = a.embed_scale[tok] * (float)static_cast<const int8_t*>(a.embed)[(long long)tok * D + d] + a.dec_pos[(long long)pos * D + d];
      else
        a.dx[i] = e2f(static_cast<const bf16*>(a.embed)[(long long)tok * D + d]) + a.dec_pos[(long long)pos * D + d];
    }
  }
  bar.sync();

  const int nph = a.L * 6;
  for (int ph = 0; ph < nph; ++ph) {
    const int l = ph / 6, g = ph - l * 6;
    const MegaLayer& L = sl[l];
    {
      const int n = cur.n0 + warp * cur.R;
      const bool active = n < cur.nend;
      float res = 0.f;
      {
        const int m = lane & 7, r_sel = lane >> 3;
        if (cur.residual && active && r_sel < cur.R && m < MB && m < Q && n + r_sel < cur.nend)
          res = __ldcg(cur.residual + (long long)m * cur.ldo + n + r_sel);
      }
      auto ahead = [&]() {
        if (dbuf && ph + 1 < nph) {
          const GemvDesc d1 = make_desc<VAR, W8>(a, sl, (ph + 1) / 6, (ph + 1) % 6, pos);
          issue_slabs<ESZ>(d1, pool + (((ph + 1) & 1) ? 0 : a.p0_off), &cbar[(ph + 1) & 1]);
        }
        if (g == 0 && threadIdx.x == DMA_T + 1 && blockIdx.x < Q * H * nsplit) {
          const int item = blockIdx.x;
          const int split = item % nsplit, h = (item / nsplit) % H, q = item / (nsplit * H);
          const int s0 = split * ks;
          const int n = max(0, min(a.S, s0 + ks) - s0);
          if (n > 0) {
            l2_prefetch(L.cross_k + (((long long)q * H + h) * a.S + s0) * 64, (uint32_t)n * 128);
            l2_prefetch(L.cross_v + (((long long)q * H + h) * a.S + s0) * 64, (uint32_t)n * 128);
          }
        }
      };
      stage_x<MB, VAR>(xs, red, cur, pre, Q, split_end, a, g == 3, ahead);
      mark(2);
      if (mkbase && lane == 0) wts[warp][0] = wts[warp][1] = 0;
      if (active) {
        mbar_wait(&cbar[ph & 1], (ph & 1) ? cpar1 : cpar0);
        if (mkbase && lane == 0) wts[warp][0] = global_ns();
        const uint8_t* slab = pool + ((ph & 1) ? 0 : a.p0_off) + (size_t)warp * cur.R * cur.K * ESZ;
        float acc[RMAX][MB];
        if (cur.R == 4) dot_rows<MB, 4, W8>(slab, xs, cur.K, acc, lane);
        else if (cur.R == 3) dot_rows<MB, 3, W8>(slab, xs, cur.K, acc, lane);
        else if (cur.R == 2) dot_rows<MB, 2, W8>(slab, xs, cur.K, acc, lane);
        else dot_rows<MB, 1, W8>(slab, xs, cur.K, acc, lane);
        finish_rows<MB, VAR, W8>(cur, acc, pre.scale, pre.bias, n, Q, res, true, D, a.Tmax, pos, lane);
        if (mkbase && lane == 0) wts[warp][1] = global_ns();
      }
      mark(3);
      if (cur.n0 < cur.nend) {
        if (ph & 1) cpar1 ^= 1u;
        else cpar0 ^= 1u;
      }
    }
    __syncthreads();
    bar.arrive();
    if (mkbase && threadIdx.x == 0 && bar.epoch < MEGA_TRACE_N) {
      long long t0 = 0, t1 = 0;
      for (int w = 0; w < MW; ++w) {
        t0 = wts[w][0] > t0 ? wts[w][0] : t0;
        t1 = wts[w][1] > t1 ? wts[w][1] : t1;
      }
      mkbase[bar.epoch * 4 + 0] = t0;
      mkbase[bar.epoch * 4 + 1] = t1;
    }
    cur = make_desc<VAR, W8>(a, sl, ph + 1 < nph ? (ph + 1) / 6 : a.L, (ph + 1) % 6, pos);
    if (!dbuf && !cur.lm) issue_slabs<ESZ>(cur, pool, &cbar[(ph + 1) & 1]);
    prefetch_phase<W8>(cur, pre, pool, &wbar[warp], gw, warp, lane);

    if (g == 0) {
      if (blockIdx.x < Q * H) {
        const int q = blockIdx.x / H, h = blockIdx.x - q * H;
        uint8_t* sK = att;
        uint8_t* sV = att + (size_t)MAXKEYS * 128;
        for (int s = grp; s < pos; s += KG) {
          const long long off = ((long long)q * a.Tmax + s) * D + h * 64 + sub * 8;
          cp_async16m(sK + s * 128 + sub * 16, L.self_k + off);
          cp_async16m(sV + s * 128 + sub * 16, L.self_v + off);
        }
      }
      bar.wait();
      for (int item = blockIdx.x; item < Q * H; item += gridDim.x) {
        const int q = item / H, h = item - q * H;
        const int n = pos + 1;
        uint8_t* sK = att;
        uint8_t* sV = att + (size_t)MAXKEYS * 128;
        float* redo = reinterpret_cast<float*>(att + (size_t)MAXKEYS * 256);
        const int s_first = (item == blockIdx.x) ? pos : 0;
        for (int s = s_first + grp; s < n; s += KG) {
          const long long off = ((long long)q * a.Tmax + s) * D + h * 64 + sub * 8;
          cp_async16m(sK + s * 128 + sub * 16, L.self_k + off);
          cp_async16m(sV + s * 128 + sub * 16, L.self_v + off);
        }
        float qv[8];
        {
          const float4 q0 = __ldcg(reinterpret_cast<const float4*>(a.dqkv + (long long)q * 3 * D + h * 64 + sub * 8));
          const float4 q1 = __ldcg(reinterpret_cast<const float4*>(a.dqkv + (long long)q * 3 * D + h * 64 + sub * 8 + 4));
          qv[0] = q0.x; qv[1] = q0.y; qv[2] = q0.z; qv[3] = q0.w; qv[4] = q1.x; qv[5] = q1.y; qv[6] = q1.z; qv[7] = q1.w;
        }
        cp_async_wait_allm();
        __syncthreads();
        float mx, sum, ov;
        if (n <= 3 * KG) attend_smem<3>(sK, sV, redo, red, qv, n, nullptr, mx, sum, ov);
        else attend_smem<(MAXKEYS + KG - 1) / KG>(sK, sV, redo, red, qv, n, nullptr, mx, sum, ov);
        if (threadIdx.x < 64) a.dattn[(long long)q * D + h * 64 + threadIdx.x] = ov / sum;
        fence_proxy_async_smem();
        __syncthreads();
      }
      bar.sync();
    } else if (g == 2) {
      if (threadIdx.x == 0 && blockIdx.x < Q * H * nsplit) {
        const int item = blockIdx.x;
        const int split = item % nsplit, h = (item / nsplit) % H, q = item / (nsplit * H);
        const int s0 = split * ks;
        const int n = max(0, min(a.S, s0 + ks) - s0);
        mbar_arrive_expect_tx(&xbar, (uint32_t)n * 256);
        if (n > 0) {
          bulk_g2s(att, L.cross_k + (((long long)q * H + h) * a.S + s0) * 64, (uint32_t)n * 128, &xbar);
          bulk_g2s(att + XKMAX * 128, L.cross_v + (((long long)q * H + h) * a.S + s0) * 64, (uint32_t)n * 128, &xbar);
        }
      }
      bar.wait();
      {
        uint8_t* sK = att;
        uint8_t* sV = att + XKMAX * 128;
        float* redo = reinterpret_cast<float*>(att + 2 * XKMAX * 128);
        for (int item = blockIdx.x; item < Q * H * nsplit; item += gridDim.x) {
          const int split = item % nsplit;
          const int h = (item / nsplit) % H;
          const int q = item / (nsplit * H);
          const int s0 = split * ks;
          const int n = max(0, min(a.S, s0 + ks) - s0);
          if (item != blockIdx.x && threadIdx.x == 0) {
            mbar_arrive_expect_tx(&xbar, (uint32_t)n * 256);
            if (n > 0) {
              bulk_g2s(sK, L.cross_k + (((long long)q * H + h) * a.S + s0) * 64, (uint32_t)n * 128, &xbar);
              bulk_g2s(sV, L.cross_v + (((long long)q * H + h) * a.S + s0) * 64, (uint32_t)n * 128, &xbar);
            }
          }
          float qv[8];
          {
            const float4 q0 = __ldcg(reinterpret_cast<const float4*>(a.dq + (long long)q * D + h * 64 + sub * 8));
            const float4 q1 = __ldcg(reinterpret_cast<const float4*>(a.dq + (long long)q * D + h * 64 + sub * 8 + 4));
            qv[0] = q0.x; qv[1] = q0.y; qv[2] = q0.z; qv[3] = q0.w; qv[4] = q1.x; qv[5] = q1.y; qv[6] = q1.z; qv[7] = q1.w;
          }
          float* align_row = nullptr;
          if (a.align && L.head_slots) {
            const int slot = L.head_slots[h];
            const int step = pos - a.step_base;
            if (slot >= 0 && step >= 0 && step < a.Tcap) align_row = a.align + (((long long)q * a.Ha + slot) * a.Tcap + step) * a.S + s0;
          }
          mbar_wait(&xbar, xpar);
          xpar ^= 1u;
          mark(0);
          if (mkbase && threadIdx.x == 0 && bar.epoch < MEGA_TRACE_N) mkbase[bar.epoch * 4 + 2] = clock64();
          float mx, sum, ov;
          attend_smem<(XKMAX + KG - 1) / KG>(sK, sV, redo, red, qv, n, align_row, mx, sum, ov,
                                             (mkbase && bar.epoch < MEGA_TRACE_N) ? mkbase + bar.epoch * 4 : nullptr);
          const long long pb = ((long long)q * H + h) * nsplit + split;
          if (threadIdx.x < 64) a.part_o[pb * 64 + threadIdx.x] = ov;
          if (threadIdx.x == 0) {
            a.part_ml[pb * 2 + 0] = mx;
            a.part_ml[pb * 2 + 1] = sum;
          }
          fence_proxy_async_smem();
          __syncthreads();
        }
      }
      bar.sync();
    } else {
      bar.wait();
    }
  }

  stage_x<MB, VAR>(xs, red, cur, pre, Q, split_end, a, false, [] {});
  unsigned long long best = 0ull;
  {
    const int K = cur.K, N = cur.N;
    const size_t slab_bytes = (size_t)2 * K * ESZ;
    const size_t set_bytes = slab_bytes * MW;
    int buf = 0;
    const bool at_begin = (pos + 1 == a.begin_index) && a.begin_suppress_bits;
    for (int n = gw * 2; n < N; n += GW * 2) {
      const int n2 = n + GW * 2;
      if (n2 < N) {
        __syncwarp();
        issue_rows<ESZ>(pool + (buf ^ 1) * set_bytes + (size_t)warp * slab_bytes, &wbar[(buf ^ 1) * MW + warp], cur.W, K, 2, n2, N, lane);
      }
      float sc = 1.f;
      if constexpr (W8) sc = cur.scale[min(n + (lane >> 3), N - 1)];
      if (buf == 0) {
        mbar_wait(&wbar[warp], wpar);
        wpar ^= 1u;
      } else {
        mbar_wait(&wbar[MW + warp], wpar1);
        wpar1 ^= 1u;
      }
      float acc[RMAX][MB];
      dot_rows<MB, 2, W8>(pool + buf * set_bytes + (size_t)warp * slab_bytes, xs, K, acc, lane);
      finish_rows<MB, VAR, W8>(cur, acc, sc, 0.f, n, Q, 0.f, true, D, a.Tmax, pos, lane);
      if (a.fuse_select) {
        const int m = lane & 7, r_sel = lane >> 3, nn = n + r_sel;
        if (r_sel < 2 && m < MB && m < Q && nn < N) {
          float v = 0.f;
#pragma unroll
          for (int r = 0; r < 2; ++r)
#pragma unroll
            for (int mm = 0; mm < MB; ++mm)
              if (r == r_sel && mm == m) v = acc[r][mm];
          if (W8) v *= sc;
          bool masked = (a.suppress_bits[nn >> 5] >> (nn & 31)) & 1u;
          if (at_begin) masked = masked || ((a.begin_suppress_bits[nn >> 5] >> (nn & 31)) & 1u);
          if (!masked) {
            unsigned u = __float_as_uint(v);
            u = (u & 0x80000000u) ? ~u : (u | 0x80000000u);
            const unsigned long long key = ((unsigned long long)u << 32) | (unsigned long long)(0xffffffffu - (unsigned)nn);
            best = key > best ? key : best;
          }
        }
      }
      buf ^= 1;
    }
  }
  if (a.fuse_select) {
    {
      const unsigned long long o = __shfl_xor_sync(0xffffffffu, best, 8);
      best = o > best ? o : best;
    }
    unsigned long long* sb = reinterpret_cast<unsigned long long*>(xs);
    __syncthreads();
    if (lane < MB) sb[lane * MW + warp] = best;
    __syncthreads();
    if (threadIdx.x < MB && threadIdx.x < Q) {
      unsigned long long b = 0ull;
      for (int w = 0; w < MW; ++w) b = sb[threadIdx.x * MW + w] > b ? sb[threadIdx.x * MW + w] : b;
      if (b) atomicMax(a.sel_best + threadIdx.x, b);
    }
    __syncthreads();
    if (threadIdx.x == 0) {
      const unsigned prev = atom_acq_rel_add(a.sel_ctr, 1u);
      if (prev == gridDim.x - 1) {
        const int cur_len = pos + 1;
        const bool generating = cur_len >= a.begin_index && cur_len < a.Tmax;
        for (int q = 0; q < Q; ++q) {
          const unsigned long long b = __ldcg(a.sel_best + q);
          a.sel_best[q] = 0ull;
          if (generating) {
            int choice = (int)(0xffffffffu - (unsigned)(b & 0xffffffffull));
            if (a.finished[q]) choice = a.pad;
            else if (choice == a.eos) a.finished[q] = 1;
            a.tokens_rw[q * a.Tmax + cur_len] = choice;
          }
        }
        *a.sel_ctr = 0u;
        *a.pos_rw = pos + 1;
      }
    }
  }
  if (TRACE && a.trace && bar.epoch < MEGA_TRACE_N) {
    __syncthreads();
    if (threadIdx.x == 0) a.trace[((long long)blockIdx.x * MEGA_TRACE_N + bar.epoch) * 2] = global_ns();
  }
}

}

int g_mega_coop = -1;

namespace {

template <int MB, unsigned VAR, bool W8>
int launch_mega(cudaStream_t st, const MegaArgs& a, int num_sms, int coop) {
  static size_t limit = 0, attr = 0;
  if (!limit) {
    int dev = 0, optin = 0;
    BW_CUDA_OK(cudaGetDevice(&dev));
    BW_CUDA_OK(cudaDeviceGetAttribute(&optin, cudaDevAttrMaxSharedMemoryPerBlockOptin, dev));
    cudaFuncAttributes fa{};
    BW_CUDA_OK(cudaFuncGetAttributes(&fa, decode_mega_kernel<MB, VAR, W8>));
    limit = (size_t)optin - fa.sharedSizeBytes;
  }
  MegaArgs b = a;
  const size_t smem = mega_smem_plan(MB, a.D, a.ffn, num_sms, !(a.flags & 2), limit, &b.p0_off, W8 ? 1 : 2);
  if (!smem) return -3;
  if (smem > attr) {
    BW_CUDA_OK(cudaFuncSetAttribute(decode_mega_kernel<MB, VAR, W8>, cudaFuncAttributeMaxDynamicSharedMemorySize, (int)smem));
    int per_sm = 0;
    BW_CUDA_OK(cudaOccupancyMaxActiveBlocksPerMultiprocessor(&per_sm, decode_mega_kernel<MB, VAR, W8>, MT, smem));
    if (per_sm < 1) return -3;
    attr = smem;
  }
  BW_CUDA_OK(cudaMemsetAsync(a.bar, 0, 1024 * sizeof(unsigned), st));
  cudaLaunchConfig_t cfg{};
  cfg.gridDim = dim3(num_sms); cfg.blockDim = dim3(MT); cfg.dynamicSmemBytes = smem; cfg.stream = st;
  cudaLaunchAttribute at[1];
  at[0].id = cudaLaunchAttributeCooperative; at[0].val.cooperative = 1;
  cfg.attrs = at; cfg.numAttrs = coop ? 1 : 0;
  BW_CUDA_OK(cudaLaunchKernelEx(&cfg, decode_mega_kernel<MB, VAR, W8>, b));
  return 0;
}

}

int launch_decode_mega(cudaStream_t st, const MegaArgs& a, int num_sms) {
  const int Q = a.Q;
  const bool w8 = a.embed_scale != nullptr;
  const size_t esz = w8 ? 1 : 2;
  if (a.L > MEGA_MAXL || Q > 2 || a.D > MAXD || a.ffn > 5120 || a.D % 8 != 0 || a.ffn % 8 != 0 || a.Tmax > MAXKEYS) return -3;
  if ((size_t)MW * a.D * esz > (size_t)ATT_OFF) return -3;
  {
    const int nmax = 3 * a.D > a.ffn ? 3 * a.D : a.ffn;
    if (((nmax + num_sms - 1) / num_sms + MW - 1) / MW > RMAX) return -3;
  }
  if (a.nsplit > XSPLIT) return -3;
  if ((size_t)((a.D + num_sms - 1) / num_sms) * a.D * esz > (size_t)ATT_OFF) return -3;
  const int ks = (a.S + a.nsplit - 1) / a.nsplit;
  if (ks > XKMAX) return -3;
  int& coop = g_mega_coop;
  if (coop < 0) {
    const char* ev = getenv("BW_MEGA_COOP");
    coop = (ev && ev[0] == '0') ? 0 : 1;
  }
  int rc;
  if (w8) {
    if (Q <= 1) rc = a.trace ? launch_mega<1, 0u, true>(st, a, num_sms, coop) : launch_mega<1, V_NOTRACE, true>(st, a, num_sms, coop);
    else rc = a.trace ? launch_mega<2, 0u, true>(st, a, num_sms, coop) : launch_mega<2, V_NOTRACE, true>(st, a, num_sms, coop);
  } else {
    if (Q <= 1) rc = a.trace ? launch_mega<1, 0u, false>(st, a, num_sms, coop) : launch_mega<1, V_NOTRACE, false>(st, a, num_sms, coop);
    else rc = a.trace ? launch_mega<2, 0u, false>(st, a, num_sms, coop) : launch_mega<2, V_NOTRACE, false>(st, a, num_sms, coop);
  }
  if (rc) return rc;
  BW_CUDA_OK(cudaGetLastError());
  return 0;
}

}
```

thewhisper_b200/csrc/decode_mega_common.cuh:

```cuda
#pragma once
#include <math.h>

#include "decode.cuh"
#include "kernels.h"

namespace BW_NS {
namespace mega {

constexpr int MT = 384;
constexpr int MW = MT / 32;
constexpr int RMAX = 4;
constexpr int DMA_T = MT - 32;
constexpr int KG = MT / 8;
constexpr int MAXKEYS = 448;
constexpr int XKMAX = 256;
constexpr int MAXD = 1280;
constexpr int ATT_OFF = 32 * 1024;

__device__ __forceinline__ void unpack8m(const uint4& u, float (&f)[8]) {
  float2 t;
  t = unpack_bf16(u.x); f[0] = t.x; f[1] = t.y;
  t = unpack_bf16(u.y); f[2] = t.x; f[3] = t.y;
  t = unpack_bf16(u.z); f[4] = t.x; f[5] = t.y;
  t = unpack_bf16(u.w); f[6] = t.x; f[7] = t.y;
}
__device__ __forceinline__ void cp_async16m(void* smem_dst, const void* gmem_src) {
  asm volatile("cp.async.cg.shared.global [%0], [%1], 16;" ::"r"(smem_u32(smem_dst)), "l"(gmem_src) : "memory");
}
__device__ __forceinline__ void cp_async_wait_allm() { asm volatile("cp.async.wait_all;" ::: "memory"); }
__device__ __forceinline__ void bulk_g2s(void* smem_dst, const void* gmem_src, uint32_t bytes, uint64_t* bar) {
  asm volatile("cp.async.bulk.shared::cluster.global.mbarrier::complete_tx::bytes [%0], [%1], %2, [%3];" ::"r"(smem_u32(smem_dst)),
               "l"(gmem_src), "r"(bytes), "r"(smem_u32(bar))
               : "memory");
}
__device__ __forceinline__ unsigned ld_acquire_u32(const unsigned* p) {
  unsigned v;
  asm volatile("ld.acquire.gpu.global.u32 %0, [%1];" : "=r"(v) : "l"(p) : "memory");
  return v;
}
__device__ __forceinline__ void red_release_add(unsigned* p, unsigned v) {
  asm volatile("red.release.gpu.global.add.u32 [%0], %1;" ::"l"(p), "r"(v) : "memory");
}
__device__ __forceinline__ unsigned atom_acq_rel_add(unsigned* p, unsigned v) {
  unsigned old;
  asm volatile("atom.acq_rel.gpu.global.add.u32 %0, [%1], %2;" : "=r"(old) : "l"(p), "r"(v) : "memory");
  return old;
}
__device__ __forceinline__ long long global_ns() {
  long long t;
  asm volatile("mov.u64 %0, %globaltimer;" : "=l"(t));
  return t;
}

template <int ESZ>
__device__ __forceinline__ void issue_rows(uint8_t* slab, uint64_t* bar, const uint8_t* W, int K, int R, int n, int N, int lane) {
  if (lane == 0) {
    const uint32_t row_bytes = (uint32_t)K * ESZ;
    mbar_arrive_expect_tx(bar, row_bytes * R);
    for (int r = 0; r < R; ++r) {
      const int row = min(n + r, N - 1);
      if constexpr (ESZ == 2) bulk_g2s(slab + (size_t)r * row_bytes, reinterpret_cast<const bf16*>(W) + (long long)row * K, row_bytes, bar);
      else bulk_g2s(slab + (size_t)r * row_bytes, W + (long long)row * K, row_bytes, bar);
    }
  }
}

__device__ __forceinline__ void l2_prefetch(const void* p, uint32_t bytes) {
  asm volatile("cp.async.bulk.prefetch.L2.global [%0], %1;" ::"l"(p), "r"(bytes) : "memory");
}
template <int MB, int R, bool W8>
__device__ __forceinline__ void dot_chunk(const uint8_t* slab, const float* xs, int K, int k0, bool hi, float (&s)[R][MB]) {
  float4 x0[MB], x1[MB];
#pragma unroll
  for (int m = 0; m < MB; ++m) {
    x0[m] = *reinterpret_cast<const float4*>(&xs[m * K + k0]);
    x1[m] = hi ? *reinterpret_cast<const float4*>(&xs[m * K + k0 + 128]) : make_float4(0.f, 0.f, 0.f, 0.f);
  }
#pragma unroll
  for (int r = 0; r < R; ++r) {
    float2 a0, a1, c0, c1;
    if constexpr (W8) {
      const uint32_t wa = *reinterpret_cast<const uint32_t*>(slab + (size_t)r * K + k0);
      const uint32_t wc = hi ? *reinterpret_cast<const uint32_t*>(slab + (size_t)r * K + k0 + 128) : 0u;
      float fa[4], fc[4];
      unpack_s8x4(wa, fa);
      unpack_s8x4(wc, fc);
      a0 = make_float2(fa[0], fa[1]); a1 = make_float2(fa[2], fa[3]); c0 = make_float2(fc[0], fc[1]); c1 = make_float2(fc[2], fc[3]);
    } else {
      const uint2 wa = *reinterpret_cast<const uint2*>(slab + ((size_t)r * K + k0) * 2);
      const uint2 wc = hi ? *reinterpret_cast<const uint2*>(slab + ((size_t)r * K + k0 + 128) * 2) : make_uint2(0u, 0u);
      a0 = unpack_bf16(wa.x); a1 = unpack_bf16(wa.y); c0 = unpack_bf16(wc.x); c1 = unpack_bf16(wc.y);
    }
#pragma unroll
    for (int m = 0; m < MB; ++m) {
      float t = s[r][m], u = 0.f;
      t = fmaf(a0.x, x0[m].x, t); u = fmaf(c0.x, x1[m].x, u);
      t = fmaf(a0.y, x0[m].y, t); u = fmaf(c0.y, x1[m].y, u);
      t = fmaf(a1.x, x0[m].z, t); u = fmaf(c1.x, x1[m].z, u);
      t = fmaf(a1.y, x0[m].w, t); u = fmaf(c1.y, x1[m].w, u);
      s[r][m] = t + u;
    }
  }
}

template <int MB, int R, bool W8>
__device__ __forceinline__ void dot_rows(const uint8_t* slab, const float* xs, int K, float (&acc)[RMAX][MB], int lane) {
  float s[R][MB];
#pragma unroll
  for (int r = 0; r < R; ++r)
#pragma unroll
    for (int m = 0; m < MB; ++m) s[r][m] = 0.f;
  const int nfull = K >> 8;
  int k0 = lane * 4;
#pragma unroll 5
  for (int c = 0; c < nfull; ++c, k0 += 256) dot_chunk<MB, R, W8>(slab, xs, K, k0, true, s);
  if (k0 < K) dot_chunk<MB, R, W8>(slab, xs, K, k0, (k0 + 128) < K, s);
#pragma unroll
  for (int r = 0; r < RMAX; ++r)
#pragma unroll
    for (int m = 0; m < MB; ++m) acc[r][m] = (r < R) ? warp_sum(s[r < R ? r : 0][m]) : 0.f;
}

template <int NV>
__device__ __forceinline__ float treduce(float (&v)[NV], int lane) {
  int n = NV;
#pragma unroll
  for (int m = 16; m >= 1; m >>= 1) {
    if (n > 1) {
      const int h = n >> 1;
      const bool up = (lane & m) != 0;
#pragma unroll
      for (int j = 0; j < NV / 2; ++j) {
        if (j < h) {
          const float keep = up ? v[j + h] : v[j];
          const float send = up ? v[j] : v[j + h];
          v[j] = keep + __shfl_xor_sync(0xffffffffu, send, m);
        }
      }
      n = h;
    } else {
      v[0] += __shfl_xor_sync(0xffffffffu, v[0], m);
    }
  }
  return v[0];
}

template <int NJ>
__device__ __forceinline__ void attend_smem(const uint8_t* sK, const uint8_t* sV, float* redo, float* red, const float (&qv)[8], int n,
                                            float* score_out, float& mx_out, float& sum_out, float& ov_out, long long* mk = nullptr) {
  const int grp = threadIdx.x >> 3, sub = threadIdx.x & 7;
  const int warp = threadIdx.x >> 5, lane = threadIdx.x & 31;
  float d[NJ];
#pragma unroll
  for (int j = 0; j < NJ; ++j) {
    const int kk = grp + j * KG;
    float t0 = 0.f, t1 = 0.f;
    if (kk < n) {
      float kf[8];
      unpack8m(*reinterpret_cast<const uint4*>(sK + kk * 128 + sub * 16), kf);
#pragma unroll
      for (int i = 0; i < 4; ++i) {
        t0 = fmaf(qv[i], kf[i], t0);
        t1 = fmaf(qv[i + 4], kf[i + 4], t1);
      }
    }
    d[j] = t0 + t1;
  }
#pragma unroll
  for (int st = 1; st < 8; st <<= 1) {
#pragma unroll
    for (int j = 0; j < NJ; ++j) d[j] += __shfl_xor_sync(0xffffffffu, d[j], st);
  }
  float lmax = -INFINITY;
#pragma unroll
  for (int j = 0; j < NJ; ++j) {
    const int kk = grp + j * KG;
    if (kk < n) {
      lmax = fmaxf(lmax, d[j]);
      if (score_out && sub == 0) score_out[kk] = d[j];
    }
  }
  lmax = warp_max(lmax);
  if (mk && threadIdx.x == 0) { mk[1] = global_ns(); mk[3] = clock64(); }
  if (lane == 0) red[warp] = lmax;
  __syncthreads();
  float mx = red[0];
#pragma unroll
  for (int w = 1; w < MW; ++w) mx = fmaxf(mx, red[w]);
  float acc[8], lsum = 0.f;
#pragma unroll
  for (int i = 0; i < 8; ++i) acc[i] = 0.f;
  {
    float mine = 0.f, mine2 = 0.f;
#pragma unroll
    for (int j = 0; j < NJ; ++j)
      if ((j & 7) == sub) {
        if (j < 8) mine = d[j];
        else mine2 = d[j];
      }
    mine = __expf(mine - mx);
    if (NJ > 8) mine2 = __expf(mine2 - mx);
    const int gl = lane & 24;
#pragma unroll
    for (int j = 0; j < NJ; ++j) {
      const float e = __shfl_sync(0xffffffffu, j < 8 ? mine : mine2, gl + (j & 7));
      d[j] = (grp + j * KG < n) ? e : 0.f;
    }
  }
#pragma unroll
  for (int j = 0; j < NJ; ++j) {
    const int kk = grp + j * KG;
    if (kk < n) {
      lsum += d[j];
      float vf[8];
      unpack8m(*reinterpret_cast<const uint4*>(sV + kk * 128 + sub * 16), vf);
#pragma unroll
      for (int i = 0; i < 8; ++i) acc[i] = fmaf(d[j], vf[i], acc[i]);
    }
  }
#pragma unroll
  for (int i = 0; i < 8; ++i) {
    acc[i] += __shfl_xor_sync(0xffffffffu, acc[i], 8);
    acc[i] += __shfl_xor_sync(0xffffffffu, acc[i], 16);
  }
  lsum += __shfl_xor_sync(0xffffffffu, lsum, 8);
  lsum += __shfl_xor_sync(0xffffffffu, lsum, 16);
  if (lane < 8) {
#pragma unroll
    for (int i = 0; i < 8; ++i) redo[warp * 72 + lane * 8 + i] = acc[i];
    if (lane == 0) redo[warp * 72 + 64] = lsum;
  }
  __syncthreads();
  float ov = 0.f, ls = 0.f;
#pragma unroll
  for (int w = 0; w < MW; ++w) ls += redo[w * 72 + 64];
  if (threadIdx.x < 64) {
#pragma unroll
    for (int w = 0; w < MW; ++w) ov += redo[w * 72 + threadIdx.x];
  }
  mx_out = mx;
  sum_out = ls;
  ov_out = ov;
}

inline size_t mega_smem_plan(int mb, int D, int ffn, int num_sms, bool want_dbuf, size_t limit, int* p0_off, int esz = 2) {
  auto rc = [&](int n) {
    const int rows = (n + num_sms - 1) / num_sms, R = (rows + MW - 1) / MW;
    return (size_t)((rows + R - 1) / R * R);
  };
  const size_t attn = (size_t)MAXKEYS * 256 + (size_t)(MW * 72) * sizeof(float);
  const size_t xattn = (size_t)2 * XKMAX * 128 + (size_t)(MW * 72) * sizeof(float);
  const size_t att = ATT_OFF + (attn > xattn ? attn : xattn);
  const size_t lm = (size_t)MW * 2 * 2 * D * esz;
  size_t r1 = rc(D) * ffn * esz;
  if (rc(D) * D * esz > r1) r1 = rc(D) * D * esz;
  size_t r0 = rc(3 * D) * D * esz;
  if (rc(ffn) * D * esz > r0) r0 = rc(ffn) * D * esz;
  if (rc(D) * D * esz > r0) r0 = rc(D) * D * esz;
  const size_t fixed = 64 * sizeof(float) + (size_t)mb * ffn * sizeof(float) + 128;
  auto mx = [](size_t a, size_t b) { return a > b ? a : b; };
  const size_t off = (r1 + 127) / 128 * 128;
  const size_t pool_d = mx(mx(off + r0, att), lm);
  if (want_dbuf && fixed + pool_d <= limit) {
    *p0_off = (int)off;
    return fixed + pool_d;
  }
  *p0_off = 0;
  const size_t single = fixed + mx(mx(mx(r0, r1), att), lm);
  return single <= limit ? single : 0;
}

}
}
```

Baseline: 849.3.

## Batch forced-prefix decode steps into one multi-token megakernel pass

Adds a prefix mode to the decode megakernel that handles several forced prompt tokens (up to four rows in total across beams) in a single launch. The rows are stacked as extra GEMV rows, and the KV cache is written at successive positions. Self-attention and cross-attention are run per row, while the final LM head is computed only for the last row. This cuts the number of sequential megakernel launches and weight reads for the initial forced tokens, at the cost of new template instantiations, larger shared memory for reductions, and a separately captured graph for each (Q, n) pair.

```diff
diff --git a/thewhisper_b200/csrc/api.cu b/thewhisper_b200/csrc/api.cu
--- a/thewhisper_b200/csrc/api.cu
+++ b/thewhisper_b200/csrc/api.cu
@@ -110,6 +110,7 @@
   int max_graphs = 64;
   cudaGraphExec_t cur_graph = nullptr;
   std::map<cudaGraphExec_t, int> graph_kernels;
+  std::map<std::pair<int, int>, cudaGraphExec_t> prefix_graphs;
   long long step_kernel_launches = 0;
   bool no_graph = false, simt = false, no_mega = false, no_fused_select = false;
   int mega_flags = MEGA_DEFAULT_FLAGS;
@@ -383,44 +384,52 @@
 
 __global__ void set_pos_kernel(int* pos, int v) { *pos = v; }
 
+void mega_args(bw_engine* e, MegaArgs& m) {
+  const int D = e->D, H = e->H, S = e->S, ffn = e->cfg.ffn, V = e->V, Tmax = e->Tmax, Q = e->Q;
+  const long long self_layer0 = (long long)e->cfg.max_audios * e->cfg.max_beams * Tmax * D;
+  const long long cross_layer0 = (long long)e->cfg.max_audios * H * S * 64;
+  m = MegaArgs{};
+  for (size_t l = 0; l < e->dec.size(); ++l) {
+    const DecLayer& L = e->dec[l];
+    MegaLayer& o = m.layers[l];
+    o.ln1g = L.ln1g; o.ln1b = L.ln1b; o.bqkv = L.bqkv; o.bo = L.bo; o.ln2g = L.ln2g; o.ln2b = L.ln2b; o.xbq = L.xbq; o.xbo = L.xbo;
+    o.ln3g = L.ln3g; o.ln3b = L.ln3b; o.b1 = L.b1; o.b2 = L.b2;
+    o.wqkv = L.wqkv; o.wo = L.wo; o.xwq = L.xwq; o.xwo = L.xwo; o.w1 = L.w1; o.w2 = L.w2;
+    o.self_k = e->self_k + l * self_layer0; o.self_v = e->self_v + l * self_layer0;
+    o.cross_k = e->cross_k + l * cross_layer0; o.cross_v = e->cross_v + l * cross_layer0;
+    o.head_slots = (e->opts.record_alignment && e->cfg.n_align_heads > 0) ? e->head_slots + l * H : nullptr;
+  }
+  m.L = (int)e->dec.size(); m.D = D; m.H = H; m.ffn = ffn; m.V = V; m.S = S; m.Tmax = Tmax; m.Q = Q;
+  m.embed = e->embed; m.embed_scale = e->embed_scale; m.wscale = e->wscale_tab; m.dec_pos = e->dec_pos; m.lnf_g = e->dec_lnf_g; m.lnf_b = e->dec_lnf_b;
+  m.tokens = e->tokens; m.pos = e->pos; m.ldl = e->Vp;
+  m.dx = e->dx; m.dqkv = e->dqkv; m.dattn = e->dattn; m.dq = e->dq; m.dh = e->dh; m.logits = e->logits;
+  m.part_o = e->part_o; m.part_ml = e->part_ml; m.bar = e->mega_bar;
+  int ns = e->num_sms / (Q * H);
+  const int ns_min = (S + 255) / 256;
+  if (ns < ns_min) ns = ns_min;
+  if (ns > XSPLIT) ns = XSPLIT;
+  m.nsplit = ns;
+  if (e->opts.record_alignment && e->cfg.n_align_heads > 0) {
+    m.align = e->align; m.Ha = e->cfg.n_align_heads; m.Tcap = e->cfg.max_align_steps; m.step_base = e->opts.begin_index;
+  }
+  m.trace = e->mega_trace;
+  if (!e->opts.timestamp_rules && !e->no_fused_select && !e->scores) {
+    m.fuse_select = 1;
+    m.suppress_bits = e->sup_bits; m.begin_suppress_bits = e->bsup_bits; m.begin_index = e->opts.begin_index;
+    m.eos = e->opts.eos_token; m.pad = e->opts.pad_token; m.finished = e->finished; m.tokens_rw = e->tokens; m.pos_rw = e->pos;
+    m.sel_best = e->sel_best; m.sel_ctr = e->sel_ctr;
+  }
+  m.flags = e->mega_flags;
+}
+
+bool mega_applies(const bw_engine* e) { return !e->no_mega && !e->has_k0 && e->G == 1 && e->Q <= 8 && (int)e->dec.size() <= MEGA_MAXL; }
+
 int step_impl(bw_engine* e, cudaStream_t st) {
   const int D = e->D, H = e->H, S = e->S, ffn = e->cfg.ffn, V = e->V, Tmax = e->Tmax, Q = e->Q, A = e->A, G = e->G;
-  const long long self_layer0 = (long long)e->cfg.max_audios * e->cfg.max_beams * Tmax * D;
-  const long long cross_layer0 = (long long)e->cfg.max_audios * H * S * 64;
   bool mega_done = false, select_done = false;
-  if (!e->no_mega && !e->has_k0 && G == 1 && Q <= 8 && (int)e->dec.size() <= MEGA_MAXL) {
-    MegaArgs m{};
-    for (size_t l = 0; l < e->dec.size(); ++l) {
-      const DecLayer& L = e->dec[l];
-      MegaLayer& o = m.layers[l];
-      o.ln1g = L.ln1g; o.ln1b = L.ln1b; o.bqkv = L.bqkv; o.bo = L.bo; o.ln2g = L.ln2g; o.ln2b = L.ln2b; o.xbq = L.xbq; o.xbo = L.xbo;
-      o.ln3g = L.ln3g; o.ln3b = L.ln3b; o.b1 = L.b1; o.b2 = L.b2;
-      o.wqkv = L.wqkv; o.wo = L.wo; o.xwq = L.xwq; o.xwo = L.xwo; o.w1 = L.w1; o.w2 = L.w2;
-      o.self_k = e->self_k + l * self_layer0; o.self_v = e->self_v + l * self_layer0;
-      o.cross_k = e->cross_k + l * cross_layer0; o.cross_v = e->cross_v + l * cross_layer0;
-      o.head_slots = (e->opts.record_alignment && e->cfg.n_align_heads > 0) ? e->head_slots + l * H : nullptr;
-    }
-    m.L = (int)e->dec.size(); m.D = D; m.H = H; m.ffn = ffn; m.V = V; m.S = S; m.Tmax = Tmax; m.Q = Q;
-    m.embed = e->embed; m.embed_scale = e->embed_scale; m.wscale = e->wscale_tab; m.dec_pos = e->dec_pos; m.lnf_g = e->dec_lnf_g; m.lnf_b = e->dec_lnf_b;
-    m.tokens = e->tokens; m.pos = e->pos; m.ldl = e->Vp;
-    m.dx = e->dx; m.dqkv = e->dqkv; m.dattn = e->dattn; m.dq = e->dq; m.dh = e->dh; m.logits = e->logits;
-    m.part_o = e->part_o; m.part_ml = e->part_ml; m.bar = e->mega_bar;
-    int ns = e->num_sms / (Q * H);
-    const int ns_min = (S + 255) / 256;
-    if (ns < ns_min) ns = ns_min;
-    if (ns > XSPLIT) ns = XSPLIT;
-    m.nsplit = ns;
-    if (e->opts.record_alignment && e->cfg.n_align_heads > 0) {
-      m.align = e->align; m.Ha = e->cfg.n_align_heads; m.Tcap = e->cfg.max_align_steps; m.step_base = e->opts.begin_index;
-    }
-    m.trace = e->mega_trace;
-    if (!e->opts.timestamp_rules && !e->no_fused_select && !e->scores) {
-      m.fuse_select = 1;
-      m.suppress_bits = e->sup_bits; m.begin_suppress_bits = e->bsup_bits; m.begin_index = e->opts.begin_index;
-      m.eos = e->opts.eos_token; m.pad = e->opts.pad_token; m.finished = e->finished; m.tokens_rw = e->tokens; m.pos_rw = e->pos;
-      m.sel_best = e->sel_best; m.sel_ctr = e->sel_ctr;
-    }
-    m.flags = e->mega_flags;
+  if (mega_applies(e)) {
+    MegaArgs m;
+    mega_args(e, m);
     const int rc = launch_decode_mega(st, m, e->num_sms);
     if (rc == 0) {
       mega_done = true;
@@ -630,6 +639,8 @@
 void bw_engine_destroy(bw_engine* e) {
   if (!e) return;
   for (auto& kv : e->graphs) cudaGraphExecDestroy(kv.second);
+  for (auto& kv : e->prefix_graphs)
+    if (kv.second) cudaGraphExecDestroy(kv.second);
   for (auto& kv : e->enc_graphs) cudaGraphExecDestroy(kv.second);
   for (auto& kv : e->buffers) cudaFree(kv.second.first);
   logmel_plan_destroy(e->mel_plan);
@@ -751,11 +762,12 @@
   if (dalloc(e, "sel_best", &e->sel_best, (size_t)Qm)) return -1;
   if (dalloc(e, "sup_bits", &e->sup_bits, (size_t)(V + 31) / 32)) return -1;
   if (dalloc(e, "bsup_bits", &e->bsup_bits, (size_t)(V + 31) / 32)) return -1;
-  if (dalloc(e, "dx", &e->dx, (size_t)Qm * D)) return -1;
-  if (dalloc(e, "dqkv", &e->dqkv, (size_t)Qm * 3 * D)) return -1;
-  if (dalloc(e, "dattn", &e->dattn, (size_t)Qm * D)) return -1;
-  if (dalloc(e, "dq", &e->dq, (size_t)Qm * D)) return -1;
-  if (dalloc(e, "dh", &e->dh, (size_t)Qm * c.ffn)) return -1;
+  const size_t Qr = Qm > 4 ? Qm : 4;
+  if (dalloc(e, "dx", &e->dx, Qr * D)) return -1;
+  if (dalloc(e, "dqkv", &e->dqkv, Qr * 3 * D)) return -1;
+  if (dalloc(e, "dattn", &e->dattn, Qr * D)) return -1;
+  if (dalloc(e, "dq", &e->dq, Qr * D)) return -1;
+  if (dalloc(e, "dh", &e->dh, Qr * c.ffn)) return -1;
   if (dalloc(e, "logits", &e->logits, (size_t)Qm * e->Vp)) return -1;
   {
     const size_t qpad = ((size_t)Qm + 127) / 128 * 128;
@@ -771,8 +783,8 @@
   if (dalloc(e, "run_scores", &e->run_scores, (size_t)Qm)) return -1;
   if (dalloc(e, "cand_scores", &e->cand_scores, (size_t)Qm * 16)) return -1;
   if (dalloc(e, "cand_tokens", &e->cand_tokens, (size_t)Qm * 16)) return -1;
-  if (dalloc(e, "part_o", &e->part_o, (size_t)A * H * XSPLIT * c.max_beams * 64)) return -1;
-  if (dalloc(e, "part_ml", &e->part_ml, (size_t)A * H * XSPLIT * c.max_beams * 2)) return -1;
+  if (dalloc(e, "part_o", &e->part_o, Qr * H * XSPLIT * 64)) return -1;
+  if (dalloc(e, "part_ml", &e->part_ml, Qr * H * XSPLIT * 2)) return -1;
   if (dalloc(e, "head_slots", &e->head_slots, (size_t)c.dec_layers * H)) return -1;
   {
     std::vector<int> hs((size_t)c.dec_layers * H, -1);
@@ -930,6 +942,52 @@
   return 0;
 }
 
+static int capture_graph(bw_engine* e, int (*enqueue)(bw_engine*, cudaStream_t, int), int arg, cudaGraphExec_t* out, int* n_kernel_nodes) {
+  cudaStream_t cs;
+  BW_CUDA_OK(cudaStreamCreateWithFlags(&cs, cudaStreamNonBlocking));
+  cudaGraph_t graph = nullptr;
+  for (int attempt = 0; attempt < 2; ++attempt) {
+    BW_CUDA_OK(cudaStreamBeginCapture(cs, cudaStreamCaptureModeThreadLocal));
+    const int rc = enqueue(e, cs, arg);
+    const cudaError_t ce = cudaStreamEndCapture(cs, &graph);
+    if (rc == 0 && ce == cudaSuccess) break;
+    if (graph) cudaGraphDestroy(graph);
+    graph = nullptr;
+    cudaGetLastError();
+    if (rc == -3 && ce == cudaSuccess) {
+      cudaStreamDestroy(cs);
+      return -3;
+    }
+    if (attempt == 0 && (g_mega_coop == 1 || g_pdl_enabled == 1)) {
+      g_mega_coop = 0;
+      g_pdl_enabled = 0;
+      continue;
+    }
+    cudaStreamDestroy(cs);
+    if (rc == 0) set_error("cudaStreamEndCapture: %s", cudaGetErrorString(ce));
+    return -1;
+  }
+  *n_kernel_nodes = 0;
+  {
+    size_t nn = 0;
+    if (cudaGraphGetNodes(graph, nullptr, &nn) == cudaSuccess && nn > 0) {
+      std::vector<cudaGraphNode_t> nodes(nn);
+      if (cudaGraphGetNodes(graph, nodes.data(), &nn) == cudaSuccess) {
+        for (size_t i = 0; i < nn; ++i) {
+          cudaGraphNodeType ty;
+          if (cudaGraphNodeGetType(nodes[i], &ty) == cudaSuccess && ty == cudaGraphNodeTypeKernel) ++*n_kernel_nodes;
+        }
+      }
+    }
+  }
+  *out = nullptr;
+  const cudaError_t ie = cudaGraphInstantiate(out, graph, 0);
+  cudaGraphDestroy(graph);
+  cudaStreamDestroy(cs);
+  BW_CUDA_OK(ie);
+  return 0;
+}
+
 static int acquire_step_graph(bw_engine* e) {
   e->graph_pending = false;
   const bw_decode_opts* opts = &e->opts;
@@ -952,44 +1010,10 @@
         ++e->graph_evictions;
       }
       const auto t_capture = std::chrono::steady_clock::now();
-      cudaStream_t cs;
-      BW_CUDA_OK(cudaStreamCreateWithFlags(&cs, cudaStreamNonBlocking));
-      cudaGraph_t graph = nullptr;
-      for (int attempt = 0; attempt < 2; ++attempt) {
-        BW_CUDA_OK(cudaStreamBeginCapture(cs, cudaStreamCaptureModeThreadLocal));
-        const int rc = step_impl(e, cs);
-        const cudaError_t ce = cudaStreamEndCapture(cs, &graph);
-        if (rc == 0 && ce == cudaSuccess) break;
-        if (graph) cudaGraphDestroy(graph);
-        graph = nullptr;
-        cudaGetLastError();
-        if (attempt == 0 && (g_mega_coop == 1 || g_pdl_enabled == 1)) {
-          g_mega_coop = 0;
-          g_pdl_enabled = 0;
-          continue;
-        }
-        cudaStreamDestroy(cs);
-        if (rc == 0) set_error("cudaStreamEndCapture: %s", cudaGetErrorString(ce));
-        return -1;
-      }
+      cudaGraphExec_t exec = nullptr;
       int n_kernel_nodes = 0;
-      {
-        size_t nn = 0;
-        if (cudaGraphGetNodes(graph, nullptr, &nn) == cudaSuccess && nn > 0) {
-          std::vector<cudaGraphNode_t> nodes(nn);
-          if (cudaGraphGetNodes(graph, nodes.data(), &nn) == cudaSuccess) {
-            for (size_t i = 0; i < nn; ++i) {
-              cudaGraphNodeType ty;
-              if (cudaGraphNodeGetType(nodes[i], &ty) == cudaSuccess && ty == cudaGraphNodeTypeKernel) ++n_kernel_nodes;
-            }
-          }
-        }
-      }
-      cudaGraphExec_t exec = nullptr;
-      BW_CUDA_OK(cudaGraphInstantiate(&exec, graph, 0));
-      cudaGraphDestroy(graph);
+      if (int rc = capture_graph(e, [](bw_engine* e, cudaStream_t cs, int) { return step_impl(e, cs); }, 0, &exec, &n_kernel_nodes)) return rc;
       e->graph_kernels[exec] = n_kernel_nodes;
-      cudaStreamDestroy(cs);
       it = e->graphs.emplace(key, exec).first;
       ++e->graph_captures;
       e->graph_capture_us +=
@@ -998,6 +1022,35 @@
     e->graph_used[key] = ++e->graph_tick;
     e->cur_graph = it->second;
   }
+  return 0;
+}
+
+static int prefix_impl(bw_engine* e, cudaStream_t st, int n) {
+  MegaArgs m;
+  mega_args(e, m);
+  m.fuse_select = 0;
+  m.align = nullptr;
+  for (int l = 0; l < m.L; ++l) m.layers[l].head_slots = nullptr;
+  m.pos_rw = e->pos;
+  m.npass = n;
+  return launch_decode_mega(st, m, e->num_sms);
+}
+
+static int run_prefix(bw_engine* e, cudaStream_t st, int n) {
+  if (e->no_graph) return prefix_impl(e, st, n);
+  const std::pair<int, int> key(e->Q, n);
+  auto it = e->prefix_graphs.find(key);
+  if (it == e->prefix_graphs.end()) {
+    cudaGraphExec_t exec = nullptr;
+    int n_kernel_nodes = 0;
+    const int rc = capture_graph(e, prefix_impl, n, &exec, &n_kernel_nodes);
+    if (rc && rc != -3) return rc;
+    if (exec) e->graph_kernels[exec] = n_kernel_nodes;
+    it = e->prefix_graphs.emplace(key, exec).first;
+  }
+  if (!it->second) return -3;
+  BW_CUDA_OK(cudaGraphLaunch(it->second, st));
+  e->step_kernel_launches += e->graph_kernels[it->second];
   return 0;
 }
 
@@ -1008,7 +1061,19 @@
   cudaStream_t st = static_cast<cudaStream_t>(stream);
   if (n_steps > 0 && e->graph_pending)
     if (int rc = acquire_step_graph(e)) return rc;
-  for (int i = 0; i < n_steps; ++i, ++e->steps) {
+  int i = 0;
+  const int nf = e->opts.begin_index - 1;
+  if (e->steps == 0 && n_steps >= nf && nf <= mega::PFX_MAXKEYS && !e->scores && mega_applies(e) && e->Q <= 2) {
+    while (nf - e->steps >= 2) {
+      const int n = nf - e->steps < 4 / e->Q ? nf - e->steps : 4 / e->Q;
+      const int rc = run_prefix(e, st, n);
+      if (rc == -3) break;
+      if (rc) return rc;
+      e->steps += n;
+      i += n;
+    }
+  }
+  for (; i < n_steps; ++i, ++e->steps) {
     if (e->cur_graph) {
       BW_CUDA_OK(cudaGraphLaunch(e->cur_graph, st));
       e->step_kernel_launches += e->graph_kernels[e->cur_graph];
@@ -1271,9 +1336,9 @@
 }
 
 static int mega_plan(int32_t Q, int32_t D, int32_t ffn, int32_t num_sms, int32_t smem_optin, int32_t static_smem, int64_t* out, int esz) {
-  BW_CHECK(out && Q >= 1 && D > 0 && ffn > 0 && num_sms > 0 && smem_optin > static_smem, "bw_op_mega_plan: bad arguments");
+  BW_CHECK(out && Q >= 1 && Q <= 4 && D > 0 && ffn > 0 && num_sms > 0 && smem_optin > static_smem, "bw_op_mega_plan: bad arguments");
   int p0_off = 0;
-  const size_t smem = mega::mega_smem_plan(Q <= 1 ? 1 : 2, D, ffn, num_sms, true, (size_t)(smem_optin - static_smem), &p0_off, esz);
+  const size_t smem = mega::mega_smem_plan(Q, D, ffn, num_sms, true, (size_t)(smem_optin - static_smem), &p0_off, esz);
   out[0] = (int64_t)smem;
   out[1] = p0_off;
   return smem ? 0 : -3;
diff --git a/thewhisper_b200/csrc/decode.cuh b/thewhisper_b200/csrc/decode.cuh
--- a/thewhisper_b200/csrc/decode.cuh
+++ b/thewhisper_b200/csrc/decode.cuh
@@ -130,6 +130,7 @@
   int p0_off;
   const float* const* wscale;
   const float* embed_scale;
+  int npass;
 };
 
 int launch_decode_mega(cudaStream_t st, const MegaArgs& a, int num_sms);
diff --git a/thewhisper_b200/csrc/decode_mega.cu b/thewhisper_b200/csrc/decode_mega.cu
--- a/thewhisper_b200/csrc/decode_mega.cu
+++ b/thewhisper_b200/csrc/decode_mega.cu
@@ -133,7 +133,7 @@
   }
 }
 
-template <bool W8>
+template <int MB, bool W8>
 __device__ __forceinline__ void prefetch_phase(const GemvDesc& d, Pre& p, uint8_t* pool, uint64_t* wbar, int gw, int warp, int lane) {
   constexpr int ESZ = W8 ? 1 : 2;
   int n;
@@ -144,8 +144,9 @@
     n = d.n0 + warp * d.R;
   }
   const int r_sel = lane >> 3;
-  p.bias = (d.bias && (lane & 7) < 2 && r_sel < d.R && n + r_sel < d.nend) ? d.bias[n + r_sel] : 0.f;
-  if constexpr (W8) p.scale = (!d.lm && (lane & 7) < 2 && r_sel < d.R && n + r_sel < d.nend) ? d.scale[n + r_sel] : 1.f;
+  constexpr int FL = MB > 2 ? MB : 2;
+  p.bias = (d.bias && (lane & 7) < FL && r_sel < d.R && n + r_sel < d.nend) ? d.bias[n + r_sel] : 0.f;
+  if constexpr (W8) p.scale = (!d.lm && (lane & 7) < FL && r_sel < d.R && n + r_sel < d.nend) ? d.scale[n + r_sel] : 1.f;
   const int k = threadIdx.x * 4;
   if (d.lng && k < d.K) {
     p.g = *reinterpret_cast<const float4*>(d.lng + k);
@@ -249,7 +250,7 @@
 #pragma unroll
       for (int u = 0; u < U; ++u) {
         const int i = base + u * ST * 4;
-        const int m = (MB > 1 && i >= K) ? 1 : 0;
+        const int m = MB > 2 ? i / K : ((MB > 1 && i >= K) ? 1 : 0);
         v[u] = make_float4(0.f, 0.f, 0.f, 0.f);
         if (i < MB * K && m < M) v[u] = __ldcg(reinterpret_cast<const float4*>(d.src + (long long)m * K + (i - m * K)));
       }
@@ -314,7 +315,7 @@
 
 template <int MB, unsigned VAR, bool W8>
 __device__ __forceinline__ void finish_rows(const GemvDesc& d, const float (&acc)[RMAX][MB], float scale, float bias, int n, int M,
-                                            float res, bool res_valid, int D, int Tmax, int pos, int lane) {
+                                            float res, bool res_valid, int D, int Tmax, int pos, int nq, int lane) {
   const int m = lane & 7, r_sel = lane >> 3;
   const int nn = n + r_sel;
   if (r_sel < d.R && m < MB && m < M && nn < d.nend) {
@@ -332,7 +333,7 @@
     if (d.residual) v += res_valid ? res : __ldcg(d.residual + (long long)m * d.ldo + nn);
     d.out[(long long)m * d.ldo + nn] = v;
     if (d.kc && nn >= D) {
-      const long long row = ((long long)m * Tmax + pos) * D;
+      const long long row = MB > 2 ? ((long long)(m % nq) * Tmax + pos + m / nq) * D : ((long long)m * Tmax + pos) * D;
       if (nn < 2 * D) d.kc[row + nn - D] = f2e(v);
       else d.vc[row + nn - 2 * D] = f2e(v);
     }
@@ -343,9 +344,12 @@
 __global__ void __launch_bounds__(MT, 1) decode_mega_kernel(const __grid_constant__ MegaArgs a) {
   constexpr bool TRACE = !(VAR & V_NOTRACE);
   constexpr int ESZ = W8 ? 1 : 2;
+  constexpr bool PFX = MB > 2;
+  constexpr int MBL = PFX ? (MB == 3 ? 1 : 2) : MB;
+  constexpr int SKEYS = PFX ? PFX_MAXKEYS : MAXKEYS;
   extern __shared__ __align__(128) uint8_t dyn[];
   float* red = reinterpret_cast<float*>(dyn);
-  float* xs = red + 64;
+  float* xs = red + red_floats(MB);
   uint8_t* pool = reinterpret_cast<uint8_t*>(xs + (size_t)MB * a.ffn);
   uint8_t* att = pool + ATT_OFF;
   __shared__ __align__(8) uint64_t wbar[2 * MW];
@@ -357,6 +361,8 @@
   const int warp = threadIdx.x >> 5, lane = threadIdx.x & 31;
   const int gw = blockIdx.x * MW + warp, GW = gridDim.x * MW;
   const int D = a.D, H = a.H, Q = a.Q;
+  const int np = PFX ? a.npass : 1;
+  const int M = PFX ? Q * np : Q;
   const int pos0 = *a.pos;
   GridBar<VAR> bar{a.bar, gridDim.x, 0u, a.trace};
   const bool split_end = (a.flags & 64) != 0;
@@ -390,15 +396,16 @@
   Pre pre;
   const bool dbuf = a.p0_off > 0;
   issue_slabs<ESZ>(cur, pool + a.p0_off, &cbar[0]);
-  prefetch_phase<W8>(cur, pre, pool, &wbar[warp], gw, warp, lane);
+  prefetch_phase<MB, W8>(cur, pre, pool, &wbar[warp], gw, warp, lane);
   if (blockIdx.x == 0) {
-    for (int i = threadIdx.x; i < Q * D; i += MT) {
-      const int q = i / D, d = i - q * D;
-      const int tok = a.tokens[q * a.Tmax + pos];
+    for (int i = threadIdx.x; i < M * D; i += MT) {
+      const int m = i / D, d = i - m * D;
+      const int q = PFX ? m % Q : m, p = PFX ? pos + m / Q : pos;
+      const int tok = a.tokens[q * a.Tmax + p];
       if constexpr (W8)
-        a.dx[i] = a.embed_scale[tok] * (float)static_cast<const int8_t*>(a.embed)[(long long)tok * D + d] + a.dec_pos[(long long)pos * D + d];
+        a.dx[i] = a.embed_scale[tok] * (float)static_cast<const int8_t*>(a.embed)[(long long)tok * D + d] + a.dec_pos[(long long)p * D + d];
       else
-        a.dx[i] = e2f(static_cast<const bf16*>(a.embed)[(long long)tok * D + d]) + a.dec_pos[(long long)pos * D + d];
+        a.dx[i] = e2f(static_cast<const bf16*>(a.embed)[(long long)tok * D + d]) + a.dec_pos[(long long)p * D + d];
     }
   }
   bar.sync();
@@ -413,7 +420,7 @@
       float res = 0.f;
       {
         const int m = lane & 7, r_sel = lane >> 3;
-        if (cur.residual && active && r_sel < cur.R && m < MB && m < Q && n + r_sel < cur.nend)
+        if (cur.residual && active && r_sel < cur.R && m < MB && m < M && n + r_sel < cur.nend)
           res = __ldcg(cur.residual + (long long)m * cur.ldo + n + r_sel);
       }
       auto ahead = [&]() {
@@ -432,7 +439,7 @@
           }
         }
       };
-      stage_x<MB, VAR>(xs, red, cur, pre, Q, split_end, a, g == 3, ahead);
+      stage_x<MB, VAR>(xs, red, cur, pre, M, split_end, a, g == 3, ahead);
       mark(2);
       if (mkbase && lane == 0) wts[warp][0] = wts[warp][1] = 0;
       if (active) {
@@ -444,7 +451,7 @@
         else if (cur.R == 3) dot_rows<MB, 3, W8>(slab, xs, cur.K, acc, lane);
         else if (cur.R == 2) dot_rows<MB, 2, W8>(slab, xs, cur.K, acc, lane);
         else dot_rows<MB, 1, W8>(slab, xs, cur.K, acc, lane);
-        finish_rows<MB, VAR, W8>(cur, acc, pre.scale, pre.bias, n, Q, res, true, D, a.Tmax, pos, lane);
+        finish_rows<MB, VAR, W8>(cur, acc, pre.scale, pre.bias, n, M, res, true, D, a.Tmax, pos, Q, lane);
         if (mkbase && lane == 0) wts[warp][1] = global_ns();
       }
       mark(3);
@@ -466,13 +473,14 @@
     }
     cur = make_desc<VAR, W8>(a, sl, ph + 1 < nph ? (ph + 1) / 6 : a.L, (ph + 1) % 6, pos);
     if (!dbuf && !cur.lm) issue_slabs<ESZ>(cur, pool, &cbar[(ph + 1) & 1]);
-    prefetch_phase<W8>(cur, pre, pool, &wbar[warp], gw, warp, lane);
+    prefetch_phase<MB, W8>(cur, pre, pool, &wbar[warp], gw, warp, lane);
 
     if (g == 0) {
-      if (blockIdx.x < Q * H) {
-        const int q = blockIdx.x / H, h = blockIdx.x - q * H;
+      if (blockIdx.x < M * H) {
+        const int m = blockIdx.x / H, h = blockIdx.x - m * H;
+        const int q = PFX ? m % Q : m;
         uint8_t* sK = att;
-        uint8_t* sV = att + (size_t)MAXKEYS * 128;
+        uint8_t* sV = att + (size_t)SKEYS * 128;
         for (int s = grp; s < pos; s += KG) {
           const long long off = ((long long)q * a.Tmax + s) * D + h * 64 + sub * 8;
           cp_async16m(sK + s * 128 + sub * 16, L.self_k + off);
@@ -480,12 +488,13 @@
         }
       }
       bar.wait();
-      for (int item = blockIdx.x; item < Q * H; item += gridDim.x) {
-        const int q = item / H, h = item - q * H;
-        const int n = pos + 1;
+      for (int item = blockIdx.x; item < M * H; item += gridDim.x) {
+        const int m = item / H, h = item - m * H;
+        const int q = PFX ? m % Q : m;
+        const int n = (PFX ? pos + m / Q : pos) + 1;
         uint8_t* sK = att;
-        uint8_t* sV = att + (size_t)MAXKEYS * 128;
-        float* redo = reinterpret_cast<float*>(att + (size_t)MAXKEYS * 256);
+        uint8_t* sV = att + (size_t)SKEYS * 128;
+        float* redo = reinterpret_cast<float*>(att + (size_t)SKEYS * 256);
         const int s_first = (item == blockIdx.x) ? pos : 0;
         for (int s = s_first + grp; s < n; s += KG) {
           const long long off = ((long long)q * a.Tmax + s) * D + h * 64 + sub * 8;
@@ -494,16 +503,16 @@
         }
         float qv[8];
         {
-          const float4 q0 = __ldcg(reinterpret_cast<const float4*>(a.dqkv + (long long)q * 3 * D + h * 64 + sub * 8));
-          const float4 q1 = __ldcg(reinterpret_cast<const float4*>(a.dqkv + (long long)q * 3 * D + h * 64 + sub * 8 + 4));
+          const float4 q0 = __ldcg(reinterpret_cast<const float4*>(a.dqkv + (long long)m * 3 * D + h * 64 + sub * 8));
+          const float4 q1 = __ldcg(reinterpret_cast<const float4*>(a.dqkv + (long long)m * 3 * D + h * 64 + sub * 8 + 4));
           qv[0] = q0.x; qv[1] = q0.y; qv[2] = q0.z; qv[3] = q0.w; qv[4] = q1.x; qv[5] = q1.y; qv[6] = q1.z; qv[7] = q1.w;
         }
         cp_async_wait_allm();
         __syncthreads();
         float mx, sum, ov;
         if (n <= 3 * KG) attend_smem<3>(sK, sV, redo, red, qv, n, nullptr, mx, sum, ov);
-        else attend_smem<(MAXKEYS + KG - 1) / KG>(sK, sV, redo, red, qv, n, nullptr, mx, sum, ov);
-        if (threadIdx.x < 64) a.dattn[(long long)q * D + h * 64 + threadIdx.x] = ov / sum;
+        else attend_smem<(SKEYS + KG - 1) / KG>(sK, sV, redo, red, qv, n, nullptr, mx, sum, ov);
+        if (threadIdx.x < 64) a.dattn[(long long)m * D + h * 64 + threadIdx.x] = ov / sum;
         fence_proxy_async_smem();
         __syncthreads();
       }
@@ -538,30 +547,35 @@
               bulk_g2s(sV, L.cross_v + (((long long)q * H + h) * a.S + s0) * 64, (uint32_t)n * 128, &xbar);
             }
           }
-          float qv[8];
-          {
-            const float4 q0 = __ldcg(reinterpret_cast<const float4*>(a.dq + (long long)q * D + h * 64 + sub * 8));
-            const float4 q1 = __ldcg(reinterpret_cast<const float4*>(a.dq + (long long)q * D + h * 64 + sub * 8 + 4));
-            qv[0] = q0.x; qv[1] = q0.y; qv[2] = q0.z; qv[3] = q0.w; qv[4] = q1.x; qv[5] = q1.y; qv[6] = q1.z; qv[7] = q1.w;
-          }
-          float* align_row = nullptr;
-          if (a.align && L.head_slots) {
-            const int slot = L.head_slots[h];
-            const int step = pos - a.step_base;
-            if (slot >= 0 && step >= 0 && step < a.Tcap) align_row = a.align + (((long long)q * a.Ha + slot) * a.Tcap + step) * a.S + s0;
-          }
-          mbar_wait(&xbar, xpar);
-          xpar ^= 1u;
-          mark(0);
-          if (mkbase && threadIdx.x == 0 && bar.epoch < MEGA_TRACE_N) mkbase[bar.epoch * 4 + 2] = clock64();
-          float mx, sum, ov;
-          attend_smem<(XKMAX + KG - 1) / KG>(sK, sV, redo, red, qv, n, align_row, mx, sum, ov,
-                                             (mkbase && bar.epoch < MEGA_TRACE_N) ? mkbase + bar.epoch * 4 : nullptr);
-          const long long pb = ((long long)q * H + h) * nsplit + split;
-          if (threadIdx.x < 64) a.part_o[pb * 64 + threadIdx.x] = ov;
-          if (threadIdx.x == 0) {
-            a.part_ml[pb * 2 + 0] = mx;
-            a.part_ml[pb * 2 + 1] = sum;
+          for (int j = 0; j < np; ++j) {
+            const int m = PFX ? j * Q + q : q;
+            float qv[8];
+            {
+              const float4 q0 = __ldcg(reinterpret_cast<const float4*>(a.dq + (long long)m * D + h * 64 + sub * 8));
+              const float4 q1 = __ldcg(reinterpret_cast<const float4*>(a.dq + (long long)m * D + h * 64 + sub * 8 + 4));
+              qv[0] = q0.x; qv[1] = q0.y; qv[2] = q0.z; qv[3] = q0.w; qv[4] = q1.x; qv[5] = q1.y; qv[6] = q1.z; qv[7] = q1.w;
+            }
+            float* align_row = nullptr;
+            if (!PFX && a.align && L.head_slots) {
+              const int slot = L.head_slots[h];
+              const int step = pos - a.step_base;
+              if (slot >= 0 && step >= 0 && step < a.Tcap) align_row = a.align + (((long long)q * a.Ha + slot) * a.Tcap + step) * a.S + s0;
+            }
+            if (j == 0) {
+              mbar_wait(&xbar, xpar);
+              xpar ^= 1u;
+              mark(0);
+              if (mkbase && threadIdx.x == 0 && bar.epoch < MEGA_TRACE_N) mkbase[bar.epoch * 4 + 2] = clock64();
+            }
+            float mx, sum, ov;
+            attend_smem<(XKMAX + KG - 1) / KG>(sK, sV, redo, red, qv, n, align_row, mx, sum, ov,
+                                               (mkbase && bar.epoch < MEGA_TRACE_N) ? mkbase + bar.epoch * 4 : nullptr);
+            const long long pb = ((long long)m * H + h) * nsplit + split;
+            if (threadIdx.x < 64) a.part_o[pb * 64 + threadIdx.x] = ov;
+            if (threadIdx.x == 0) {
+              a.part_ml[pb * 2 + 0] = mx;
+              a.part_ml[pb * 2 + 1] = sum;
+            }
           }
           fence_proxy_async_smem();
           __syncthreads();
@@ -573,7 +587,8 @@
     }
   }
 
-  stage_x<MB, VAR>(xs, red, cur, pre, Q, split_end, a, false, [] {});
+  if constexpr (PFX) cur.src += (long long)(np - 1) * Q * D;
+  stage_x<MBL, VAR>(xs, red, cur, pre, Q, split_end, a, false, [] {});
   unsigned long long best = 0ull;
   {
     const int K = cur.K, N = cur.N;
@@ -596,17 +611,17 @@
         mbar_wait(&wbar[MW + warp], wpar1);
         wpar1 ^= 1u;
       }
-      float acc[RMAX][MB];
-      dot_rows<MB, 2, W8>(pool + buf * set_bytes + (size_t)warp * slab_bytes, xs, K, acc, lane);
-      finish_rows<MB, VAR, W8>(cur, acc, sc, 0.f, n, Q, 0.f, true, D, a.Tmax, pos, lane);
-      if (a.fuse_select) {
+      float acc[RMAX][MBL];
+      dot_rows<MBL, 2, W8>(pool + buf * set_bytes + (size_t)warp * slab_bytes, xs, K, acc, lane);
+      finish_rows<MBL, VAR, W8>(cur, acc, sc, 0.f, n, Q, 0.f, true, D, a.Tmax, pos, Q, lane);
+      if (!PFX && a.fuse_select) {
         const int m = lane & 7, r_sel = lane >> 3, nn = n + r_sel;
-        if (r_sel < 2 && m < MB && m < Q && nn < N) {
+        if (r_sel < 2 && m < MBL && m < Q && nn < N) {
           float v = 0.f;
 #pragma unroll
           for (int r = 0; r < 2; ++r)
 #pragma unroll
-            for (int mm = 0; mm < MB; ++mm)
+            for (int mm = 0; mm < MBL; ++mm)
               if (r == r_sel && mm == m) v = acc[r][mm];
           if (W8) v *= sc;
           bool masked = (a.suppress_bits[nn >> 5] >> (nn & 31)) & 1u;
@@ -622,16 +637,16 @@
       buf ^= 1;
     }
   }
-  if (a.fuse_select) {
+  if (!PFX && a.fuse_select) {
     {
       const unsigned long long o = __shfl_xor_sync(0xffffffffu, best, 8);
       best = o > best ? o : best;
     }
     unsigned long long* sb = reinterpret_cast<unsigned long long*>(xs);
     __syncthreads();
-    if (lane < MB) sb[lane * MW + warp] = best;
+    if (lane < MBL) sb[lane * MW + warp] = best;
     __syncthreads();
-    if (threadIdx.x < MB && threadIdx.x < Q) {
+    if (threadIdx.x < MBL && threadIdx.x < Q) {
       unsigned long long b = 0ull;
       for (int w = 0; w < MW; ++w) b = sb[threadIdx.x * MW + w] > b ? sb[threadIdx.x * MW + w] : b;
       if (b) atomicMax(a.sel_best + threadIdx.x, b);
@@ -657,6 +672,12 @@
       }
     }
   }
+  if constexpr (PFX) {
+    if (blockIdx.x == 0) {
+      for (int i = threadIdx.x; i < Q * D; i += MT) a.dx[i] = __ldcg(a.dx + (long long)(np - 1) * Q * D + i);
+      if (threadIdx.x == 0) *a.pos_rw = pos + np;
+    }
+  }
   if (TRACE && a.trace && bar.epoch < MEGA_TRACE_N) {
     __syncthreads();
     if (threadIdx.x == 0) a.trace[((long long)blockIdx.x * MEGA_TRACE_N + bar.epoch) * 2] = global_ns();
@@ -722,7 +743,11 @@
     coop = (ev && ev[0] == '0') ? 0 : 1;
   }
   int rc;
-  if (w8) {
+  if (a.npass > 0) {
+    if (a.npass < 2 || Q * a.npass > 4 || a.trace) return -3;
+    if (Q * a.npass == 4) rc = w8 ? launch_mega<4, V_NOTRACE, true>(st, a, num_sms, coop) : launch_mega<4, V_NOTRACE, false>(st, a, num_sms, coop);
+    else rc = w8 ? launch_mega<3, V_NOTRACE, true>(st, a, num_sms, coop) : launch_mega<3, V_NOTRACE, false>(st, a, num_sms, coop);
+  } else if (w8) {
     if (Q <= 1) rc = a.trace ? launch_mega<1, 0u, true>(st, a, num_sms, coop) : launch_mega<1, V_NOTRACE, true>(st, a, num_sms, coop);
     else rc = a.trace ? launch_mega<2, 0u, true>(st, a, num_sms, coop) : launch_mega<2, V_NOTRACE, true>(st, a, num_sms, coop);
   } else {
diff --git a/thewhisper_b200/csrc/decode_mega_common.cuh b/thewhisper_b200/csrc/decode_mega_common.cuh
--- a/thewhisper_b200/csrc/decode_mega_common.cuh
+++ b/thewhisper_b200/csrc/decode_mega_common.cuh
@@ -13,9 +13,11 @@
 constexpr int DMA_T = MT - 32;
 constexpr int KG = MT / 8;
 constexpr int MAXKEYS = 448;
+constexpr int PFX_MAXKEYS = 256;
 constexpr int XKMAX = 256;
 constexpr int MAXD = 1280;
 constexpr int ATT_OFF = 32 * 1024;
+constexpr int red_floats(int mb) { return mb > 2 ? 2 * mb * MW : 64; }
 
 __device__ __forceinline__ void unpack8m(const uint4& u, float (&f)[8]) {
   float2 t;
@@ -248,7 +250,7 @@
     const int rows = (n + num_sms - 1) / num_sms, R = (rows + MW - 1) / MW;
     return (size_t)((rows + R - 1) / R * R);
   };
-  const size_t attn = (size_t)MAXKEYS * 256 + (size_t)(MW * 72) * sizeof(float);
+  const size_t attn = (size_t)(mb > 2 ? PFX_MAXKEYS : MAXKEYS) * 256 + (size_t)(MW * 72) * sizeof(float);
   const size_t xattn = (size_t)2 * XKMAX * 128 + (size_t)(MW * 72) * sizeof(float);
   const size_t att = ATT_OFF + (attn > xattn ? attn : xattn);
   const size_t lm = (size_t)MW * 2 * 2 * D * esz;
@@ -257,7 +259,7 @@
   size_t r0 = rc(3 * D) * D * esz;
   if (rc(ffn) * D * esz > r0) r0 = rc(ffn) * D * esz;
   if (rc(D) * D * esz > r0) r0 = rc(D) * D * esz;
-  const size_t fixed = 64 * sizeof(float) + (size_t)mb * ffn * sizeof(float) + 128;
+  const size_t fixed = red_floats(mb) * sizeof(float) + (size_t)mb * ffn * sizeof(float) + 128;
   auto mx = [](size_t a, size_t b) { return a > b ? a : b; };
   const size_t off = (r1 + 127) / 128 * 128;
   const size_t pool_d = mx(mx(off + r0, att), lm);
```

After: 854.3, median of 6. Within noise of the previous version (+0.6%).
